# samson6460/tf2_YOLO

Hardware: AMD Instinct MI355X
Metric: images/sec training YOLOv3 416x416 bs=32/GPU (higher is better)
Workload: dtype f32-storage/fp16x2-mfma

## Files before the change

include/yolo_hip.h:

```cpp
#ifndef YOLO_HIP_H_
#define YOLO_HIP_H_

#include <stddef.h>
#include <stdint.h>

#ifdef __cplusplus
extern "C" {
#endif

typedef enum yolo_status {
  YOLO_OK = 0,
  YOLO_ERR_INVALID_ARG = -1,
  YOLO_ERR_LAUNCH = -2,
  YOLO_ERR_WORKSPACE = -3
} yolo_status;

enum { YOLO_ACT_LINEAR = 0, YOLO_ACT_LEAKY = 1, YOLO_ACT_MISH = 2 };
enum { YOLO_HEAD_V3 = 3, YOLO_HEAD_V2 = 2, YOLO_HEAD_V1 = 1, YOLO_HEAD_V4 = 4 };
enum { YOLO_NMS_HARD = 1, YOLO_NMS_SOFT = 2, YOLO_NMS_DIOU = 3 };

const char* yolo_last_error(void);
int yolo_abi_version(void);
int yolo_device_available(void);
int yolo_mfma_probe(const void* operands_f16, float* sink, int workgroups, int iters, double* flops_host, void* stream);

enum { YOLO_OPT_CONV_WIN = 0, YOLO_OPT_STAMPS = 1, YOLO_OPT_CONV_SK = 2, YOLO_OPT_CONV_PATCH = 5, YOLO_OPT_WGRAD_WIN = 6,
       YOLO_OPT_NMS_WALK = 7 ,
       YOLO_OPT_AB = 8  };
int yolo_set_option(int key, int value);
size_t yolo_conv_workspace_bytes(void);
int yolo_set_conv_workspace(void* p, size_t bytes, void* stream);
int yolo_set_debug_buffer(void* p, size_t bytes);

typedef struct yolo_conv_desc {
  int N, H, W, Cin;
  int Cout, kh, kw;
  int Ho, Wo;
  int sh, sw;
  int pad_t, pad_l;
} yolo_conv_desc;

#define YOLO_BN_STAT_SLOTS 64
#define YOLO_BN_RED_SLOTS 512
#define YOLO_SPLIT_BATCH_UNITS 4

int yolo_conv2d_fwd(const yolo_conv_desc* d, const float* x, const float* w,
                    const float* bias, float* y, double* stats, void* stream);
int yolo_conv2d_fwd_absmax(const yolo_conv_desc* d, const float* x, const float* w, const float* bias,
                           float* y, double* stats, unsigned* absmax, void* stream);

int yolo_conv2d_dgrad(const yolo_conv_desc* d, const float* dy, const float* wT,
                      float* dx, int accumulate, void* stream);

int yolo_conv2d_wgrad(const yolo_conv_desc* d, const float* x, const float* dy,
                      float* dw, float* dbias, void* stream);

int yolo_conv2d_wgrad_bias(const float* dy, long long P, int Cout, float* dbias, void* stream);

int yolo_filter_transpose(const float* w, float* wT, int Cout, int taps, int Cin, void* stream);

size_t yolo_planes_bytes(long long rows, int C);
int yolo_split_planes(const float* x, long long rows, int C, void* planes, void* stream);
int yolo_split_planes_padded(const float* x, long long rows, int C_src, int C, void* planes, void* stream);

int yolo_split_planes_batch(const void* jobs, int njobs, long long total_blocks, void* stream);
int yolo_filter_transpose_batch(const void* jobs, int njobs, long long total_blocks, void* stream);

int yolo_conv2d_fwd_planes(const yolo_conv_desc* d, const void* x_planes, const void* w_planes,
                           const float* bias, float* y, double* stats, unsigned* absmax, void* stream);
int yolo_conv2d_dgrad_planes(const yolo_conv_desc* d, const void* dy_planes, const void* wT_planes,
                             float* dx, int accumulate, void* stream);
enum { YOLO_EPI_NONE = 0, YOLO_EPI_AFFINE = 1, YOLO_EPI_AFFINE_LEAKY = 2, YOLO_EPI_AFFINE_MISH = 3 };
int yolo_conv2d_fwd_planes_epi(const yolo_conv_desc* d, const void* x_planes, const void* w_planes, const float* bias,
                               int epilogue, const float* scale, const float* shift, const float* residual, float* y,
                               unsigned* absmax, void* stream);
int yolo_split_planes_absmax(const float* x, long long rows, int C, const unsigned* absmax, const float* extra_bound,
                             void* planes, float* out_bound, void* stream);
#define YOLO_INFER_BOUND_WORDS 4096
int yolo_conv_pred_bound(const float* w, int Cout, int kdim, const float* scale, const float* shift, const float* bias,
                         float* pred2, void* stream);
int yolo_conv2d_fwd_infer_unit(const yolo_conv_desc* d, const void* x_planes, const void* w_planes, const float* bias,
                               int epilogue, const float* scale, const float* shift, const float* residual, float* y,
                               unsigned* absmax, const float* pred2, const void* in_bound, int in_n,
                               const void* residual_bound, int residual_n, void* out_planes, unsigned* out_words,
                               float* out_bound, int* out_n_host, void* stream);
int yolo_fold_bound(const void* words, int n, float* out_bound, void* stream);
int yolo_absmax_words(const float* x, long long n, unsigned* words, int* n_words_host, void* stream);
int yolo_stem_filter_prep(const float* w, const float* bias, float* wt, void* stream);
int yolo_stem_fwd_infer_unit(const yolo_conv_desc* d, const float* x, const float* wt, int epilogue, const float* scale,
                             const float* shift, const float* pred2, const void* in_bound, int in_n, float* y,
                             void* out_planes, unsigned* out_words, int* out_n_host, void* stream);
int yolo_split_planes_concat(const float* const* srcs_host, const int* channels_host, const float* const* bounds_host,
                             int nsrc, long long rows, void* planes, float* dst32, float* out_bound, void* stream);
int yolo_split_planes_concat_ex(const float* const* srcs_host, const int* channels_host, const float* const* bounds_host,
                                const int* bound_words_host, const int* upsample_host, int H, int W, int nsrc,
                                long long rows, void* planes, float* dst32, float* out_bound, void* stream);
int yolo_conv2d_fwd_head_unit(const yolo_conv_desc* d, const void* x_planes, const void* w_planes, const float* bias,
                              int A, int C, int version, const float* anchors, float* t, float* y, void* stream);
int yolo_conv2d_wgrad_planes(const yolo_conv_desc* d, const void* x_planes, const void* dy_planes,
                             float* dw, void* stream);

size_t yolo_wgrad_workspace_bytes(void);
int yolo_set_wgrad_workspace(void* p, size_t bytes);


int yolo_bn_stats(const float* x, long long P, int C, double* stats, void* stream);

int yolo_bn_finalize(double* stats, long long P, int C, const float* gamma, const float* beta,
                     float eps, float momentum, int unbiased_moving_var,
                     float* moving_mean, float* moving_var,
                     float* scale, float* shift, float* save_mean, float* save_invstd,
                     void* stream);

int yolo_bn_fold_inference(int C, const float* gamma, const float* beta,
                           const float* moving_mean, const float* moving_var, float eps,
                           float* scale, float* shift, void* stream);

int yolo_bn_act_fwd(const float* x, long long P, int C, const float* scale, const float* shift,
                    int act, const float* residual, float* out, void* stream);

int yolo_bn_act_bwd_reduce(const float* x, const float* dout, long long P, int C,
                           const float* scale, const float* shift,
                           const float* save_mean, const float* save_invstd,
                           int act, double* red, void* stream);
int yolo_bn_act_bwd_apply(const float* x, const float* dout, long long P, int C,
                          const float* gamma, const float* scale, const float* shift,
                          const float* save_mean, const float* save_invstd,
                          int act, double* red, float* dgamma, float* dbeta,
                          float* dx, void* stream);

int yolo_bn_finalize_bound(double* stats, long long P, int C, const float* gamma, const float* beta, float eps,
                           float momentum, int unbiased_moving_var, float* moving_mean, float* moving_var,
                           float* scale, float* shift, float* save_mean, float* save_invstd,
                           const unsigned* absmax, unsigned* bound, void* stream);
int yolo_bn_finalize_offset(double* stats, long long P, int C, const float* gamma, const float* beta, float eps,
                            float momentum, int unbiased_moving_var, float* moving_mean, float* moving_var, float* scale,
                            float* shift, float* save_mean, float* save_invstd, const unsigned* absmax, unsigned* bound,
                            const float* mean_offset, void* stream);
int yolo_bn_infer_bound(int C, const float* scale, const float* shift, const unsigned* absmax,
                        unsigned* bound, void* stream);
int yolo_bn_act_fwd_planes(const float* x, long long P, int C, const float* scale, const float* shift,
                           int act, const float* residual, float* out, void* planes,
                           const unsigned* bn_bound, const float* residual_bound, float* out_bound,
                           void* stream);
int yolo_bn_act_maxpool2x2_fwd(const float* y, int N, int Ho, int Wo, int C, const float* scale, const float* shift,
                               int act, float* out, int* argmax, void* planes, const unsigned* bn_bound,
// ... 3 lines not shown
                               float* out_bound, void* stream);
int yolo_bn_act_bwd_reduce_bound(const float* x, const float* dout, long long P, int C, const float* scale,
                                 const float* shift, const float* save_mean, const float* save_invstd,
                                 int act, double* red, unsigned* bound_aux, void* stream);
size_t yolo_stem_bwd_scratch_bytes(void);
int yolo_stem_bn_bwd_wgrad(const yolo_conv_desc* d, const float* y, const float* dout, const float* image, const float* scale,
                           const float* shift, const float* save_mean, const float* save_invstd, int act, const double* red,
                           float* dgamma, float* dbeta, float* dw, void* scratch, size_t scratch_bytes, void* stream);
int yolo_bn_act_bwd_apply_planes(const float* x, const float* dout, long long P, int C, const float* gamma,
                                 const float* scale, const float* shift, const float* save_mean,
                                 const float* save_invstd, int act, double* red, float* dgamma, float* dbeta,
                                 float* dx, void* planes, const unsigned* bound_aux, void* stream);
int yolo_bn_act_bwd_reduce_bound_ld(const float* x, const float* dout, long long ld_dout, long long P, int C,
                                    const float* scale, const float* shift, const float* save_mean,
                                    const float* save_invstd, int act, double* red, unsigned* bound_aux, void* stream);
#define YOLO_BN_FOLD_TICKET_WORDS 36
int yolo_bn_act_bwd_reduce_fold_ld(const float* x, const float* dout, long long ld_dout, long long P, int C,
                                   const float* scale, const float* shift, const float* save_mean,
                                   const float* save_invstd, int act, double* red, unsigned* bound_aux,
                                   unsigned* tickets, void* stream);
int yolo_bn_act_bwd_apply_planes_ld(const float* x, const float* dout, long long ld_dout, long long P, int C,
                                    const float* gamma, const float* scale, const float* shift, const float* save_mean,
                                    const float* save_invstd, int act, double* red, float* dgamma, float* dbeta,
                                    float* dx, void* planes, const unsigned* bound_aux, void* stream);

int yolo_bnred_slots_cap(const yolo_conv_desc* d);
int yolo_conv2d_dgrad_planes_bnred(const yolo_conv_desc* d, const void* dy_planes, const void* wT_planes, float* dx,
                                   int accumulate, const float* y, const float* scale, const float* shift,
                                   const float* save_mean, const float* save_invstd, int act, float* partials,
                                   int slots_cap, unsigned* bound_aux, int* nslots, void* stream);
int yolo_bn_act_bwd_sum_partials(const float* partials, int nslots, long long P, int C, const float* scale, double* red,
                                 unsigned* bound_aux, void* stream);

int yolo_act_fwd(const float* x, long long n, int act, float* out, void* stream);
int yolo_act_bwd(const float* x, const float* dout, long long n, int act, float* dx, void* stream);

int yolo_copy_channels_in(const float* src, long long P, int Csrc, float* dst, int Cdst,
                          int c_off, void* stream);
int yolo_copy_channels_out(const float* src, long long P, int Csrc, int c_off, float* dst,
                           int Cdst, int accumulate, void* stream);
int yolo_upsample2x_fwd(const float* x, int N, int H, int W, int C, float* y, int Cy, int c_off,
                        void* stream);
int yolo_upsample2x_bwd(const float* dy, int N, int H, int W, int C, int Cy, int c_off, float* dx,
                        int accumulate, void* stream);
int yolo_axpy(float* a, const float* b, long long n, void* stream);
int yolo_maxpool_fwd(const float* x, int N, int H, int W, int C, int k, int s, int pad_t, int pad_l,
                     int Ho, int Wo, float* y, int Cy, int c_off, int* argmax, void* stream);
int yolo_maxpool_bwd(const float* dy, int N, int Ho, int Wo, int C, int Cy, int c_off,
                     const int* argmax, float* dx, void* stream);
int yolo_maxpool_bwd_same(const float* dy, int N, int H, int W, int C, int Cy, int c_off, const int* argmax, int k,
                          int pad_t, int pad_l, float* dx, void* stream);
int yolo_maxpool2x2_bwd(const float* dy, int N, int Ho, int Wo, int C, const int* argmax, float* dx, int accumulate,
                        void* stream);
int yolo_space_to_depth2_fwd(const float* x, int N, int H, int W, int C, float* y, int Cy, int c_off,
                             void* stream);
int yolo_space_to_depth2_bwd(const float* dy, int N, int H, int W, int C, int Cy, int c_off, float* dx,
                             int accumulate, void* stream);

int yolo_head_act_fwd(const float* t, long long P, int A, int C, int version,
                      const float* anchors, float* y, void* stream);
int yolo_head_act_bwd(const float* y, const float* dy, long long P, int A, int C, int version,
                      const float* anchors, float* dt, float* danchors, void* stream);

typedef struct yolo_loss_cfg {
  int version;
  int N, gh, gw, A, C;
  float anchors[32];
  int   use_anchors;
  float binary_weight;
  float loss_weight[4];
  float ignore_thresh;
  int   use_focal_loss;
  float focal_gamma;
  int   use_scale;
  float wh_reg_weight;
  float truth_thresh;
  float label_smooth;
} yolo_loss_cfg;

size_t yolo_loss_workspace_bytes(const yolo_loss_cfg* cfg);
int yolo_loss_fwd_bwd(const yolo_loss_cfg* cfg, const float* y_true, const float* y_pred,
                      double* loss_out, float* dpred, float grad_scale,
                      void* workspace, size_t workspace_bytes, void* stream);

int yolo_metrics(const yolo_loss_cfg* cfg, const float* y_true, const float* y_pred,
                 float recall_thresh, double* out, void* stream);

int yolo_adam_step(float* p, float* g, float* m, float* v, long long n, float lr, float beta1,
                   float beta2, float eps, int step, float grad_scale, int zero_grad, void* stream);
float yolo_adam_lr_t(float lr, float beta1, float beta2, int step);
int yolo_adam_step_dev(float* p, float* g, float* m, float* v, long long n, const float* hyper, int zero_grad, void* stream);
int yolo_sgd_step(float* p, float* g, long long n, float lr, float grad_scale, int zero_grad,
                  void* stream);
int yolo_fill(float* p, long long n, float value, void* stream);

size_t yolo_grad_sqnorm_workspace_bytes(int n_chunks);
int yolo_grad_sqnorm(const float* g, const long long* chunk_off, const int* chunk_len, int n_chunks,
                     const int* var_first, int n_vars, double* var_sq, double* total_sq, void* workspace,
                     size_t workspace_bytes, void* stream);
int yolo_clip_factors(const double* var_sq, int n_vars, const double* total_sq, const double* total_sq_extra,
                      const float* hyper, int mode, float* factors, float* norm_out, void* stream);
int yolo_adam_step_clip(float* p, float* g, float* m, float* v, float* vhat, const long long* chunk_off,
                        const int* chunk_len, const int* chunk_var, int n_chunks, const float* hyper,
                        const float* factors, int clip_mode, int zero_grad, void* stream);
int yolo_sgd_step_clip(float* p, float* g, float* accum, int nesterov, const long long* chunk_off,
                       const int* chunk_len, const int* chunk_var, int n_chunks, const float* hyper,
                       const float* factors, int clip_mode, int zero_grad, void* stream);

int yolo_decode_level(const float* pred, int gh, int gw, int A, int C, int version,
                      float threshold, double* rows_out, int max_rows, int* count,
                      void* workspace, size_t workspace_bytes, void* stream);
int yolo_decode_level_f64(const double* pred, int gh, int gw, int A, int C, int version,
                          double threshold, double* rows_out, int max_rows, int* count,
                          void* workspace, size_t workspace_bytes, void* stream);
size_t yolo_decode_workspace_bytes(int gh, int gw, int A, int C);

size_t yolo_nms_workspace_bytes(int n, int class_num);
int yolo_nms(const double* rows, int n, int class_num, int mode, double nms_threshold,
             double conf_threshold, double sigma, unsigned char* keep_out,
             void* workspace, size_t workspace_bytes, void* stream);
int yolo_nms_select(const double* rows, int n, int class_num, int mode, double nms_threshold, double conf_threshold,
                    double sigma, unsigned char* keep_out, double* rows_out, int* count_out, void* workspace,
                    size_t workspace_bytes, void* stream);

int yolo_cal_iou(const void* xywh_true, const void* xywh_pred, void* out, void* out2, int is_f64, int mode, int ndim,
                 const long long* shape_host, const long long* true_strides_host, const long long* pred_strides_host,
                 double grid_w, double grid_h, void* stream);


int yolo_match_detections(const double* gt_rows, int ngt, const double* det_rows, int ndet, int class_num,
                          double iou_threshold, int* best_gt, unsigned char* matched, double* best_iou,
                          unsigned char* gt_flags, long long* class_counts, void* stream);

int yolo_rank_desc(const double* key, const int* segment, int n, int* rank, void* stream);

size_t yolo_pr_curve_workspace_bytes(int n, int num_gts);
int yolo_pr_curve(const double* joint, const int* gt_id, const unsigned char* matched, int n, int num_gts,
                  int precision_mode, void* workspace, size_t workspace_bytes, double* precision,
                  double* recall, void* stream);

int yolo_allreduce_bucket(void* rccl_comm, float* grads, long long count, void* stream);

int yolo_encode_labels(const double* boxes, const int* cls, const int* first, int N, double img_h, double img_w,
                       int gh, int gw, int C, double* label64, float* label32, void* stream);
int yolo_down2xlabel(const double* label_in, int N, int gh, int gw, int ch, double* label_out, float* out32,
                     void* stream);

#ifdef __cplusplus
}
#endif
#endif
```

tf2_yolo_amd/_lib.py:

```python
import ctypes
import os
from ctypes import (POINTER, Structure, c_char_p, c_double, c_float, c_int, c_longlong,
                    c_size_t, c_void_p)

from . import tape as _tape

_HERE = os.path.dirname(os.path.abspath(__file__))
LIB_PATH = os.path.join(_HERE, "libyolo_hip.so")

ACT_LINEAR, ACT_LEAKY, ACT_MISH = 0, 1, 2
NMS_HARD, NMS_SOFT, NMS_DIOU = 1, 2, 3


class YoloHipError(RuntimeError):
    pass


class ConvDesc(Structure):
    _fields_ = [(n, c_int) for n in
                ("N", "H", "W", "Cin", "Cout", "kh", "kw", "Ho", "Wo", "sh", "sw", "pad_t", "pad_l")]


class LossCfg(Structure):
    _fields_ = [("version", c_int), ("N", c_int), ("gh", c_int), ("gw", c_int), ("A", c_int),
                ("C", c_int), ("anchors", c_float * 32), ("use_anchors", c_int),
                ("binary_weight", c_float), ("loss_weight", c_float * 4),
                ("ignore_thresh", c_float), ("use_focal_loss", c_int), ("focal_gamma", c_float),
                ("use_scale", c_int), ("wh_reg_weight", c_float), ("truth_thresh", c_float),
                ("label_smooth", c_float)]


_P = c_void_p
_LL = c_longlong
SIGNATURES = {
    "yolo_last_error": (c_char_p, []),
    "yolo_abi_version": (c_int, []),
    "yolo_device_available": (c_int, []),
    "yolo_set_option": (c_int, [c_int, c_int]),
    "yolo_mfma_probe": (c_int, [_P, _P, c_int, c_int, POINTER(c_double), _P]),
    "yolo_set_debug_buffer": (c_int, [_P, c_size_t]),
    "yolo_encode_labels": (c_int, [_P, _P, _P, c_int, c_double, c_double, c_int, c_int, c_int, _P, _P, _P]),
    "yolo_down2xlabel": (c_int, [_P, c_int, c_int, c_int, c_int, _P, _P, _P]),
    "yolo_conv_workspace_bytes": (c_size_t, []),
    "yolo_set_conv_workspace": (c_int, [_P, c_size_t, _P]),
    "yolo_conv2d_fwd": (c_int, [POINTER(ConvDesc), _P, _P, _P, _P, _P, _P]),
    "yolo_conv2d_dgrad": (c_int, [POINTER(ConvDesc), _P, _P, _P, c_int, _P]),
    "yolo_conv2d_wgrad": (c_int, [POINTER(ConvDesc), _P, _P, _P, _P, _P]),
    "yolo_conv2d_wgrad_bias": (c_int, [_P, _LL, c_int, _P, _P]),
    "yolo_filter_transpose": (c_int, [_P, _P, c_int, c_int, c_int, _P]),
    "yolo_planes_bytes": (c_size_t, [_LL, c_int]),
    "yolo_split_planes": (c_int, [_P, _LL, c_int, _P, _P]),
    "yolo_split_planes_padded": (c_int, [_P, _LL, c_int, c_int, _P, _P]),
    "yolo_split_planes_batch": (c_int, [_P, c_int, _LL, _P]),
    "yolo_filter_transpose_batch": (c_int, [_P, c_int, _LL, _P]),
    "yolo_conv2d_fwd_planes": (c_int, [POINTER(ConvDesc), _P, _P, _P, _P, _P, _P, _P]),
    "yolo_stem_bwd_scratch_bytes": (c_size_t, []),
    "yolo_stem_bn_bwd_wgrad": (c_int, [POINTER(ConvDesc), _P, _P, _P, _P, _P, _P, _P, c_int, _P, _P, _P, _P, _P, c_size_t, _P]),
    "yolo_conv2d_fwd_planes_epi": (c_int, [POINTER(ConvDesc), _P, _P, _P, c_int, _P, _P, _P, _P, _P, _P]),
    "yolo_split_planes_absmax": (c_int, [_P, _LL, c_int, _P, _P, _P, _P, _P]),
    "yolo_conv_pred_bound": (c_int, [_P, c_int, c_int, _P, _P, _P, _P, _P]),
    "yolo_conv2d_fwd_infer_unit": (c_int, [POINTER(ConvDesc), _P, _P, _P, c_int, _P, _P, _P, _P, _P, _P, _P, c_int, _P, c_int,
                                           _P, _P, _P, POINTER(c_int), _P]),
    "yolo_fold_bound": (c_int, [_P, c_int, _P, _P]),
    "yolo_absmax_words": (c_int, [_P, _LL, _P, POINTER(c_int), _P]),
    "yolo_stem_filter_prep": (c_int, [_P, _P, _P, _P]),
    "yolo_stem_fwd_infer_unit": (c_int, [POINTER(ConvDesc), _P, _P, c_int, _P, _P, _P, _P, c_int, _P, _P, _P, POINTER(c_int), _P]),
    "yolo_split_planes_concat": (c_int, [POINTER(c_void_p), POINTER(c_int), POINTER(c_void_p), c_int, _LL, _P, _P, _P, _P]),
    "yolo_split_planes_concat_ex": (c_int, [POINTER(c_void_p), POINTER(c_int), POINTER(c_void_p), POINTER(c_int), POINTER(c_int),
                                            c_int, c_int, c_int, _LL, _P, _P, _P, _P]),
    "yolo_conv2d_fwd_head_unit": (c_int, [POINTER(ConvDesc), _P, _P, _P, c_int, c_int, c_int, _P, _P, _P, _P]),
    "yolo_conv2d_fwd_absmax": (c_int, [POINTER(ConvDesc), _P, _P, _P, _P, _P, _P, _P]),
    "yolo_conv2d_dgrad_planes": (c_int, [POINTER(ConvDesc), _P, _P, _P, c_int, _P]),
    "yolo_conv2d_wgrad_planes": (c_int, [POINTER(ConvDesc), _P, _P, _P, _P]),
    "yolo_wgrad_workspace_bytes": (c_size_t, []),
    "yolo_set_wgrad_workspace": (c_int, [_P, c_size_t]),
    "yolo_bn_stats": (c_int, [_P, _LL, c_int, _P, _P]),
    "yolo_bn_finalize": (c_int, [_P, _LL, c_int, _P, _P, c_float, c_float, c_int, _P, _P, _P, _P, _P, _P, _P]),
    "yolo_bn_fold_inference": (c_int, [c_int, _P, _P, _P, _P, c_float, _P, _P, _P]),
    "yolo_bn_act_fwd": (c_int, [_P, _LL, c_int, _P, _P, c_int, _P, _P, _P]),
    "yolo_bn_act_bwd_reduce": (c_int, [_P, _P, _LL, c_int, _P, _P, _P, _P, c_int, _P, _P]),
    "yolo_bn_act_bwd_apply": (c_int, [_P, _P, _LL, c_int, _P, _P, _P, _P, _P, c_int, _P, _P, _P, _P, _P]),
    "yolo_bn_act_fwd_planes": (c_int, [_P, _LL, c_int, _P, _P, c_int, _P, _P, _P, _P, _P, _P, _P]),
    "yolo_bn_act_fwd_res_planes": (c_int, [_P, _LL, c_int, _P, _P, c_int, _P, _P, _P, _P, _P, _P]),
    "yolo_bn_act_bwd_apply_planes": (c_int, [_P, _P, _LL, c_int, _P, _P, _P, _P, _P, c_int, _P, _P, _P, _P, _P, _P,
                                             _P]),
    "yolo_bn_infer_bound": (c_int, [c_int, _P, _P, _P, _P, _P]),
    "yolo_bn_finalize_bound": (c_int, [_P, _LL, c_int, _P, _P, c_float, c_float, c_int, _P, _P, _P, _P, _P, _P, _P,
                                       _P, _P]),
    "yolo_bn_finalize_offset": (c_int, [_P, _LL, c_int, _P, _P, c_float, c_float, c_int, _P, _P, _P, _P, _P, _P, _P,
                                        _P, _P, _P]),
    "yolo_bn_act_bwd_reduce_bound": (c_int, [_P, _P, _LL, c_int, _P, _P, _P, _P, c_int, _P, _P, _P]),
    "yolo_bn_act_bwd_reduce_bound_ld": (c_int, [_P, _P, _LL, _LL, c_int, _P, _P, _P, _P, c_int, _P, _P, _P]),
    "yolo_bn_act_bwd_reduce_fold_ld": (c_int, [_P, _P, _LL, _LL, c_int, _P, _P, _P, _P, c_int, _P, _P, _P, _P]),
    "yolo_bn_act_bwd_apply_planes_ld": (c_int, [_P, _P, _LL, _LL, c_int, _P, _P, _P, _P, _P, c_int, _P, _P, _P, _P, _P, _P,
                                                _P]),
    "yolo_bnred_slots_cap": (c_int, [POINTER(ConvDesc)]),
    "yolo_conv2d_dgrad_planes_bnred": (c_int, [POINTER(ConvDesc), _P, _P, _P, c_int, _P, _P, _P, _P, _P, c_int, _P, c_int, _P,
                                               POINTER(c_int), _P]),
    "yolo_bn_act_bwd_sum_partials": (c_int, [_P, c_int, _LL, c_int, _P, _P, _P, _P]),
    "yolo_allreduce_bucket": (c_int, [_P, _P, _LL, _P]),
    "yolo_act_fwd": (c_int, [_P, _LL, c_int, _P, _P]),
    "yolo_act_bwd": (c_int, [_P, _P, _LL, c_int, _P, _P]),
    "yolo_copy_channels_in": (c_int, [_P, _LL, c_int, _P, c_int, c_int, _P]),
    "yolo_copy_channels_out": (c_int, [_P, _LL, c_int, c_int, _P, c_int, c_int, _P]),
    "yolo_upsample2x_fwd": (c_int, [_P, c_int, c_int, c_int, c_int, _P, c_int, c_int, _P]),
    "yolo_upsample2x_bwd": (c_int, [_P, c_int, c_int, c_int, c_int, c_int, c_int, _P, c_int, _P]),
    "yolo_axpy": (c_int, [_P, _P, _LL, _P]),
    "yolo_maxpool_fwd": (c_int, [_P, c_int, c_int, c_int, c_int, c_int, c_int, c_int, c_int, c_int, c_int,
                                 _P, c_int, c_int, _P, _P]),
    "yolo_maxpool_bwd": (c_int, [_P, c_int, c_int, c_int, c_int, c_int, c_int, _P, _P, _P]),
    "yolo_maxpool2x2_bwd": (c_int, [_P, c_int, c_int, c_int, c_int, _P, _P, c_int, _P]),
    "yolo_bn_act_maxpool2x2_fwd": (c_int, [_P, c_int, c_int, c_int, c_int, _P, _P, c_int, _P, _P, _P, _P, _P, _P]),
    "yolo_maxpool_bwd_same": (c_int, [_P, c_int, c_int, c_int, c_int, c_int, c_int, _P, c_int, c_int, c_int, _P, _P]),
    "yolo_space_to_depth2_fwd": (c_int, [_P, c_int, c_int, c_int, c_int, _P, c_int, c_int, _P]),
    "yolo_space_to_depth2_bwd": (c_int, [_P, c_int, c_int, c_int, c_int, c_int, c_int, _P, c_int, _P]),
    "yolo_head_act_fwd": (c_int, [_P, _LL, c_int, c_int, c_int, _P, _P, _P]),
    "yolo_head_act_bwd": (c_int, [_P, _P, _LL, c_int, c_int, c_int, _P, _P, _P, _P]),
    "yolo_loss_workspace_bytes": (c_size_t, [POINTER(LossCfg)]),
    "yolo_loss_fwd_bwd": (c_int, [POINTER(LossCfg), _P, _P, _P, _P, c_float, _P, c_size_t, _P]),
    "yolo_metrics": (c_int, [POINTER(LossCfg), _P, _P, c_float, _P, _P]),
    "yolo_adam_step": (c_int, [_P, _P, _P, _P, _LL, c_float, c_float, c_float, c_float, c_int, c_float, c_int, _P]),
    "yolo_adam_lr_t": (c_float, [c_float, c_float, c_float, c_int]),
    "yolo_adam_step_dev": (c_int, [_P, _P, _P, _P, _LL, _P, c_int, _P]),
    "yolo_sgd_step": (c_int, [_P, _P, _LL, c_float, c_float, c_int, _P]),
    "yolo_fill": (c_int, [_P, _LL, c_float, _P]),
    "yolo_grad_sqnorm_workspace_bytes": (c_size_t, [c_int]),
    "yolo_grad_sqnorm": (c_int, [_P, _P, _P, c_int, _P, c_int, _P, _P, _P, c_size_t, _P]),
    "yolo_clip_factors": (c_int, [_P, c_int, _P, _P, _P, c_int, _P, _P, _P]),
    "yolo_adam_step_clip": (c_int, [_P, _P, _P, _P, _P, _P, _P, _P, c_int, _P, _P, c_int, c_int, _P]),
    "yolo_sgd_step_clip": (c_int, [_P, _P, _P, c_int, _P, _P, _P, c_int, _P, _P, c_int, c_int, _P]),
    "yolo_decode_level": (c_int, [_P, c_int, c_int, c_int, c_int, c_int, c_float, _P, c_int, _P, _P, c_size_t, _P]),
    "yolo_decode_level_f64": (c_int, [_P, c_int, c_int, c_int, c_int, c_int, c_double, _P, c_int, _P, _P,
                                      c_size_t, _P]),
    "yolo_decode_workspace_bytes": (c_size_t, [c_int, c_int, c_int, c_int]),
    "yolo_nms_workspace_bytes": (c_size_t, [c_int, c_int]),
    "yolo_cal_iou": (c_int, [_P, _P, _P, _P, c_int, c_int, c_int, POINTER(c_longlong), POINTER(c_longlong),
                             POINTER(c_longlong), c_double, c_double, _P]),
    "yolo_match_detections": (c_int, [_P, c_int, _P, c_int, c_int, c_double, _P, _P, _P, _P, _P, _P]),
    "yolo_rank_desc": (c_int, [_P, _P, c_int, _P, _P]),
    "yolo_pr_curve_workspace_bytes": (c_size_t, [c_int, c_int]),
    "yolo_pr_curve": (c_int, [_P, _P, _P, c_int, c_int, c_int, _P, c_size_t, _P, _P, _P]),
    "yolo_nms": (c_int, [_P, c_int, c_int, c_int, c_double, c_double, c_double, _P, _P, c_size_t, _P]),
    "yolo_nms_select": (c_int, [_P, c_int, c_int, c_int, c_double, c_double, c_double, _P, _P, _P, _P, c_size_t, _P]),
}

_lib = None

_QUERIES = {"yolo_last_error", "yolo_abi_version", "yolo_bnred_slots_cap", "yolo_device_available", "yolo_conv_workspace_bytes", "yolo_planes_bytes",
            "yolo_stem_bwd_scratch_bytes", "yolo_loss_workspace_bytes", "yolo_decode_workspace_bytes",
            "yolo_nms_workspace_bytes", "yolo_pr_curve_workspace_bytes", "yolo_wgrad_workspace_bytes", "yolo_adam_lr_t",
            "yolo_grad_sqnorm_workspace_bytes",
            "yolo_set_option", "yolo_set_debug_buffer", "yolo_set_conv_workspace", "yolo_set_wgrad_workspace"}


class _Recorded:
    __slots__ = ("f", "name")

    def __init__(self, f, name):
        self.f, self.name = f, name

    def __call__(self, *a):
        rc = self.f(*a)
        if _tape.ACTIVE is not None:
            _tape.ACTIVE.c(self.f, a, self.name)
        return rc


class _Lib:

    def __init__(self, cdll):
        self._cdll = cdll

    def __getattr__(self, name):
        f = getattr(self._cdll, name)
        if name not in _QUERIES and name in SIGNATURES:
            f = _Recorded(f, name)
        setattr(self, name, f)
        return f


def load():
    global _lib
    if _lib is not None:
        return _lib
    if not os.path.exists(LIB_PATH):
        raise YoloHipError(
            f"{LIB_PATH} not found: build it with `make` (or __graft_entry__.build()); "
            "there is no CPU fallback for the product path")
    import torch
    try:
        lib = ctypes.CDLL(LIB_PATH)
    except OSError as e:
        raise YoloHipError(f"cannot load {LIB_PATH}: {e}") from e
    for name, (res, args) in SIGNATURES.items():
        try:
            fn = getattr(lib, name)
        except AttributeError as e:
            raise YoloHipError(f"{LIB_PATH} does not export {name}") from e
        fn.restype = res
        fn.argtypes = args
    _lib = _Lib(lib)
    return _lib
# ... 7 lines not shown
```

tf2_yolo_amd/capture.py:

```python
import torch

from ._lib import YoloHipError


_LEAKED = []


class _StaticInputs:

    def __init__(self, x, y_list):
        self.x = x.clone()
        self.ys = [y.clone() for y in y_list]
        self._last = [(x, x._version)] + [(y, y._version) for y in y_list]

    def load(self, x, y_list):
        for i, (dst, src) in enumerate(zip([self.x] + self.ys, [x] + list(y_list))):
            last, ver = self._last[i]
            if src is last and src._version == ver:
                continue
            dst.copy_(src, non_blocking=True)
            self._last[i] = (src, src._version)


class StepGraphs:

    def __init__(self, model, x, y_list):
        self.model = model
        self.key = self.key_of(model, x)
        net = model.net
        opt = model.optimizer
        if not getattr(opt, "capturable", False):
            raise YoloHipError("this optimizer has no capturable form")
        self.inputs = _StaticInputs(x, y_list)
        self.x, self.ys = self.inputs.x, self.inputs.ys
        self.segments = []
        opt._hyper_buffers()
        net.mark_params_changed()
        torch.cuda.synchronize()
        self._capture(net, opt)

    @staticmethod
    def key_of(model, x):
        return (tuple(x.shape), getattr(model.net, "alloc_gen", 0), tuple(id(l) for l in model.loss), id(model.optimizer),
                id(model._reducer), model.net.anchors_trainable)

    def _capture(self, net, opt):
        model = self.model
        red = model._reducer if (model._reducer is not None and model._reducer.active) else None
        pool = torch.cuda.graph_pool_handle()
        stream = torch.cuda.Stream()
        stream.wait_stream(torch.cuda.current_stream())
        state = {"g": None}

        def begin():
            g = torch.cuda.CUDAGraph()
            g.capture_begin(pool=pool, capture_error_mode="thread_local")
            state["g"] = g

        def end(action):
            state["g"].capture_end()
            self.segments.append((state["g"], action))
            state["g"] = None

        net._dyp_events = [None, None]
        net._wp_event = net._wT_event = None
        old_hook, old_overlap = net.grad_ready_hook, net._overlap_wgrad
        net._overlap_wgrad = False
        if red is not None:
            index = model._dp_unit_index

            def cut_hook(u):
                for b in red.closes[index[id(u)]]:
                    net._join_wgrad()
                    net._dyp_events = [None, None]
                    end(("reduce", b))
                    begin()
            net.grad_ready_hook = cut_hook
        try:
            with torch.cuda.stream(stream):
                begin()
                outs = net.forward(self.x, training=True)
                for i, (o, yt) in enumerate(zip(outs, self.ys)):
                    model.loss[i].fwd_bwd(yt, o, grad_scale=1.0, dpred=model._dpred[i], loss_out=model._loss_bufs[i])
                net.backward(model._dpred)
                net._dyp_events = [None, None]
                if red is not None:
                    end(("finish",))
                    begin()
                opt.step_captured()
                end(None)
        except Exception:
            _LEAKED.extend(g for g, _ in self.segments)
            if state["g"] is not None:
                _LEAKED.append(state["g"])
                try:
                    if net._wgrad_stream is not None:
                        torch.cuda.current_stream().wait_stream(net._wgrad_stream)
                    state["g"].capture_end()
                except Exception:
                    pass
            self.segments = []
            net._dyp_events = [None, None]
            net._wp_event = net._wT_event = None
            net._wgrad_pending = False
            raise
        finally:
            net.grad_ready_hook = old_hook
            net._overlap_wgrad = old_overlap
        torch.cuda.current_stream().wait_stream(stream)
        net.mark_params_changed()

    def replay(self, x, y_list):
        model, net, opt = self.model, self.model.net, self.model.optimizer
        red = model._reducer if (model._reducer is not None and model._reducer.active) else None
        self.inputs.load(x, y_list)
        opt.refresh_hyper(grad_scale=(1.0 / red.world) if red is not None else 1.0)
        for g, action in self.segments:
            g.replay()
            if action is None:
                continue
            if action[0] == "reduce":
                red.reduce_bucket(action[1])
            else:
                if net.anchors_trainable and red.world > 1:
                    import torch.distributed as dist
                    dist.all_reduce(net.anchor_grads, group=red.pg)
                red.finish()
        net.mark_params_changed()
        return model._loss_bufs


class StepTape:

    def __init__(self, model, x, y_list):
        from . import tape as tape_mod
        self.model = model
        self.key = StepGraphs.key_of(model, x)
        opt, net = model.optimizer, model.net
        if not getattr(opt, "capturable", False):
            raise YoloHipError("this optimizer has no capturable form")
        self.inputs = _StaticInputs(x, y_list)
        self.x, self.ys = self.inputs.x, self.inputs.ys
        opt._hyper_buffers()
        red = model._reducer if (model._reducer is not None and model._reducer.active) else None
        net._dyp_events = [None, None]
        net.mark_params_changed()
        self.tape = tape_mod.Tape()
        opt.refresh_hyper(grad_scale=(1.0 / red.world) if red is not None else 1.0)
        tape_mod.ACTIVE = self.tape
        try:
            outs = net.forward(self.x, training=True)
            for i, (o, yt) in enumerate(zip(outs, self.ys)):
                model.loss[i].fwd_bwd(yt, o, grad_scale=1.0, dpred=model._dpred[i], loss_out=model._loss_bufs[i])
            net.backward(model._dpred)
            if red is not None:
                if net.anchors_trainable and red.world > 1:
                    import torch.distributed as dist
                    tape_mod.host_call(lambda: dist.all_reduce(net.anchor_grads, group=red.pg))
                tape_mod.host_call(red.finish)
            opt.step_captured()
        finally:
            tape_mod.ACTIVE = None
        net.mark_params_changed()

    def replay(self, x, y_list):
        model, net, opt = self.model, self.model.net, self.model.optimizer
        red = model._reducer if (model._reducer is not None and model._reducer.active) else None
        self.inputs.load(x, y_list)
        opt.refresh_hyper(grad_scale=(1.0 / red.world) if red is not None else 1.0)
        self.tape.replay()
        net.mark_params_changed()
        return model._loss_bufs
```

tf2_yolo_amd/csrc/conv.hip:

```cpp
#include "conv_args.hpp"
#include <cstdlib>
#include <type_traits>

namespace yolo {

template <int BM, int BN, int WGM, int WGN, bool FLAT>
__global__ __launch_bounds__(256) void gather_conv_kernel(const GatherConvArgs a) {
  constexpr int BK = 32;
  constexpr int LD = BK + 4;
  constexpr int TM = BM / WGM / 32;
  constexpr int TN = BN / WGN / 32;
  constexpr int AR = BM / 32;
  constexpr int BR = BN / 32;
  static_assert(WGM * WGN == 4, "4 waves per block");
  static_assert(TM >= 1 && TN >= 1, "wave tile");

  extern __shared__ __attribute__((aligned(16))) float smem[];
  constexpr int BUF = (BM + BN) * LD;

  const int tid = threadIdx.x;
  const int lane = tid & 63;
  const int wave = tid >> 6;
  const int wm = wave / WGN, wn = wave % WGN;

// ... 935 lines not shown
    C += channels_host[i];
  }
  YOLO_REQUIRE((C % 16) == 0, "split_planes_concat: the concatenated channel count must be a multiple of 16");
  return launch_split_planes_concat(srcs_host, channels_host, bounds_host, nsrc, rows, planes, dst32, out_bound,
                                    as_stream(stream));
}

extern "C" int yolo_split_planes_concat_ex(const float* const* srcs_host, const int* channels_host,
                                           const float* const* bounds_host, const int* bound_words_host,
                                           const int* upsample_host, int H, int W, int nsrc, long long rows, void* planes,
                                           float* dst32, float* out_bound, void* stream) {
  YOLO_REQUIRE(srcs_host && channels_host && bounds_host && planes && nsrc >= 1 && nsrc <= 4 && rows > 0,
               "split_planes_concat: 1..4 sources, non-null tables");
  int C = 0;
  bool any_up = false;
  for (int i = 0; i < nsrc; ++i) {
    YOLO_REQUIRE(srcs_host[i] && bounds_host[i] && channels_host[i] > 0 && (channels_host[i] % 8) == 0,
                 "split_planes_concat: every source needs a pointer, a bound and a channel count that is a multiple of 8");
    YOLO_REQUIRE(bound_words_host == nullptr || (bound_words_host[i] >= 1 && bound_words_host[i] <= YOLO_INFER_BOUND_WORDS),
                 "split_planes_concat: a bound is 1..%d words", YOLO_INFER_BOUND_WORDS);
    any_up = any_up || (upsample_host != nullptr && upsample_host[i] != 0);
    C += channels_host[i];
  }
  YOLO_REQUIRE((C % 16) == 0, "split_planes_concat: the concatenated channel count must be a multiple of 16");
  YOLO_REQUIRE(!any_up || (H > 0 && W > 0 && (H % 2) == 0 && (W % 2) == 0 && rows % ((long long)H * W) == 0),
               "split_planes_concat: an upsampled source needs even H, W with rows = N * H * W (H=%d W=%d rows=%lld)", H, W, rows);
  return launch_split_planes_concat(srcs_host, channels_host, bounds_host, nsrc, rows, planes, dst32, out_bound,
                                    as_stream(stream), bound_words_host, upsample_host, H, W);
}

extern "C" int yolo_conv2d_fwd_head_unit(const yolo_conv_desc* d, const void* x_planes, const void* w_planes,
                                         const float* bias, int A, int C, int version, const float* anchors, float* t,
                                         float* y, void* stream) {
  if (int rc = validate_desc(d)) return rc;
  YOLO_REQUIRE(x_planes && w_planes && t && y && A > 0 && C > 0, "conv_fwd_head_unit: bad args");
  YOLO_REQUIRE(d->Cout == A * (5 + C), "conv_fwd_head_unit: Cout = %d is not A (5 + C) = %d", d->Cout, A * (5 + C));
  GatherConvArgs a{};
  a.src = reinterpret_cast<const float*>(x_planes);
  a.wgt = reinterpret_cast<const float*>(w_planes);
  a.bias = bias;
  a.dst = t;
  fill_fwd_args(d, a);
  YOLO_REQUIRE(gather_planes_supported(a), "conv_fwd_head_unit: needs Cin %% 16 == 0 and Cout >= 32");
  if ((version == YOLO_HEAD_V3 || version == YOLO_HEAD_V4) && anchors != nullptr) {
    a.head_y = y;
    a.head_anchors = anchors;
    a.head_A = A;
    a.head_C = C;
    if (conv_small_head_supported(a)) {
      int nwg = 0;
      return launch_conv_small(a, as_stream(stream), &nwg);
    }
    a.head_y = nullptr;
  }
  if (int rc = launch_gather_planes(a, as_stream(stream))) return rc;
  return yolo_head_act_fwd(t, (long long)d->N * d->Ho * d->Wo, A, C, version, anchors, y, stream);
}

extern "C" size_t yolo_planes_bytes(long long rows, int C) {
  if (rows <= 0 || C <= 0 || (C % 16) != 0) return 0;
  return (size_t)planes_bytes(rows, C);
}

extern "C" int yolo_split_planes_batch(const void* jobs, int njobs, long long total_blocks, void* stream) {
  YOLO_REQUIRE(jobs, "split_planes_batch: null job table");
  return launch_split_planes_batch(jobs, njobs, total_blocks, as_stream(stream));
}

extern "C" int yolo_filter_transpose_batch(const void* jobs, int njobs, long long total_blocks, void* stream) {
  YOLO_REQUIRE(jobs, "filter_transpose_batch: null job table");
  return launch_filter_transpose_batch(jobs, njobs, total_blocks, as_stream(stream));
}

extern "C" int yolo_split_planes(const float* x, long long rows, int C, void* planes, void* stream) {
  YOLO_REQUIRE(x && planes, "split_planes: null pointer");
  return launch_split_planes(x, rows, C, planes, as_stream(stream));
}

extern "C" int yolo_split_planes_padded(const float* x, long long rows, int C_src, int C, void* planes, void* stream) {
  YOLO_REQUIRE(x && planes, "split_planes_padded: null pointer");
  return launch_split_planes_padded(x, rows, C_src, C, planes, as_stream(stream));
}

struct BnRedArgs {
  const float* y;
  const float* scale;
  const float* shift;
  const float* mean;
  const float* invstd;
  int act;
  float* part;
  int cap;
  unsigned* aux;
  int nslots;
};
static void set_bnred(GatherConvArgs& a, const BnRedArgs* b) {
  if (b == nullptr) return;
  a.bwd_y = b->y; a.bwd_scale = b->scale; a.bwd_shift = b->shift; a.bwd_mean = b->mean; a.bwd_invstd = b->invstd;
  a.bwd_act = b->act; a.bwd_part = b->part; a.bwd_cap = b->cap; a.bwd_aux = b->aux;
}

static int dgrad_impl(const yolo_conv_desc* d, const float* dy, const float* wT, float* dx, int accumulate,
                      void* stream, bool planes, BnRedArgs* bnred = nullptr) {
  if (int rc = validate_desc(d)) return rc;
  YOLO_REQUIRE(dy && wT && dx, "conv_dgrad: null pointer");
  const bool flat = (d->Cout % 32) != 0;
  YOLO_REQUIRE(!flat || (d->kh == 1 && d->kw == 1 && d->sh == 1 && d->sw == 1),
               "conv_dgrad: Cout %% 32 != 0 only supported for 1x1 stride-1 (head) convs");
  static const bool fuse_classes = env_int("YOLO_DGRAD_CLASSES", 1) != 0;
  if (planes && fuse_classes && d->sh * d->sw > 1 && d->sh * d->sw <= 4) {
    GatherConvArgs a{};
    a.src = dy;
    a.wgt = wT;
    a.dst = dx;
    a.N = d->N; a.Hs = d->Ho; a.Ws = d->Wo; a.Cs = d->Cout;
    a.sy = 1; a.sx = 1;
    a.Hd = d->H; a.Wd = d->W; a.Cd = d->Cin;
    a.osy = d->sh; a.osx = d->sw;
    a.Cout = d->Cin;
    a.ldw = d->kh * d->kw * d->Cout;
    a.accumulate = accumulate;
    a.kw = 1;
    int nt = 0, nc = 0;
    bool ok = true;
    for (int py = 0; py < d->sh && ok; ++py)
      for (int px = 0; px < d->sw && ok; ++px) {
        ClassGeom& c = a.cls[nc++];
        c.Hg = (d->H - py + d->sh - 1) / d->sh;
        c.Wg = (d->W - px + d->sw - 1) / d->sw;
        c.M = (long long)d->N * c.Hg * c.Wg;
        c.ooy = py; c.oox = px; c.tap0 = nt; c.ntaps = 0;
        for (int r = 0; r < d->kh; ++r) {
          const int ty = py + d->pad_t - r;
          if (((ty % d->sh) + d->sh) % d->sh != 0) continue;
          for (int s = 0; s < d->kw; ++s) {
            const int tx = px + d->pad_l - s;
            if (((tx % d->sw) + d->sw) % d->sw != 0) continue;
            a.taps[nt++] = Tap{ty / d->sh, tx / d->sw, (r * d->kw + s) * d->Cout};
            ++c.ntaps;
          }
        }
        if (c.ntaps == 0 || c.Hg <= 0 || c.Wg <= 0) ok = false;
      }
    if (ok) {
      a.ncls = nc;
      a.M = a.cls[0].M; a.Hg = a.cls[0].Hg; a.Wg = a.cls[0].Wg; a.ooy = 0; a.oox = 0; a.ntaps = a.cls[0].ntaps;
      YOLO_REQUIRE(gather_planes_supported(a), "conv_dgrad_planes: needs Cout %% 16 == 0 and Cin >= 32");
      set_bnred(a, bnred);
      const int rc = launch_gather_planes(a, as_stream(stream));
      if (bnred != nullptr) bnred->nslots = a.bwd_nslots;
      return rc;
    }
  }
  YOLO_REQUIRE(bnred == nullptr || d->sh * d->sw == 1,
               "conv_dgrad_planes_bnred: a strided data gradient needs its parity classes in one launch");
  for (int py = 0; py < d->sh; ++py) {
    for (int px = 0; px < d->sw; ++px) {
      GatherConvArgs a{};
      a.src = dy;
      a.wgt = wT;
      a.bias = nullptr;
      a.dst = dx;
      a.N = d->N; a.Hs = d->Ho; a.Ws = d->Wo; a.Cs = d->Cout;
      a.Hg = (d->H - py + d->sh - 1) / d->sh;
      a.Wg = (d->W - px + d->sw - 1) / d->sw;
      if (a.Hg <= 0 || a.Wg <= 0) continue;
// ... 154 lines not shown
```

tf2_yolo_amd/csrc/conv_args.hpp:

```cpp
#pragma once
#include "common.hpp"

namespace yolo {

constexpr int MAX_TAPS = 49;

struct Tap {
  int oy, ox, woff;
};

struct ClassGeom {
  long long M;
  int Hg, Wg, ooy, oox, tap0, ntaps;
};

struct GatherConvArgs {
  const float* src;
  const float* wgt;
  const float* bias;
  float* dst;
  double* stats;
  unsigned* absmax;
  long long M;
  int N, Hs, Ws, Cs;
// ... 9 lines not shown
  unsigned src_bytes, wgt_bytes;
  int zero_blk_src, zero_blk_wgt;
  int nt_store;
  int vec_store;
  int kc;
  int dbg;
  const float* epi_scale;
  const float* epi_shift;
  const float* epi_res;
  int epi_act;
  unsigned char* out_planes;
  const float* pl_pred;
  const unsigned* pl_in_bound;
  const unsigned* pl_res_bound;
  int pl_in_n, pl_res_n;
  unsigned* pl_out_words;
  float* head_y;
  const float* head_anchors;
  int head_A, head_C;
  int sk_grid;
  int tile_order;
  float* sk_slabs;
  unsigned* sk_tickets;
  int split_parts;
  int ncls;
  ClassGeom cls[4];
  unsigned long long* stamps;
  const float* bwd_y;
  const float* bwd_scale;
  const float* bwd_shift;
  const float* bwd_mean;
  const float* bwd_invstd;
  float* bwd_part;
  unsigned* bwd_aux;
  int bwd_act;
  int bwd_nslots;
  int bwd_cap;
  Tap taps[MAX_TAPS];
};

#define YOLO_BNRED_CHECK(a)                                                                                          \
  if ((a).bwd_y != nullptr && (a).bwd_nslots > (a).bwd_cap) {                                                        \
    set_error("conv_dgrad(bn reduce): %d partial slots needed, room for %d", (a).bwd_nslots, (a).bwd_cap);           \
    return YOLO_ERR_INVALID_ARG;                                                                                     \
  }

__device__ __forceinline__ int xcd_remap(int bid, int nblocks) {
  const int xcd = bid & 7, idx = bid >> 3;
  const int q = nblocks >> 3, r = nblocks & 7;
  const int start = (xcd < r) ? xcd * (q + 1) : r * (q + 1) + (xcd - r) * q;
  return start + idx;
}


struct WgradArgs {
  const float* src;
  const float* dy;
  float* dw;
  long long M;
  int N, Hs, Ws, Cs;
  int Hg, Wg;
  int sy, sx;
  int Cout, ldw;
  int ntaps;
  int kw, pad_t, pad_l;
  int tiles_co, tiles_j;
  int nblocks;
  long long chunk;
  unsigned src_bytes, dy_bytes;
  int zero_blk_src, zero_blk_dy;
  float* slabs;
  int splits;
};

int launch_gather_split(GatherConvArgs& a, hipStream_t st);
bool gather_split_supported(const GatherConvArgs& a);
long long planes_bytes(long long rows, int C);
int launch_split_planes(const float* x, long long rows, int C, void* planes, hipStream_t st);
int launch_split_planes_absmax(const float* x, long long rows, int C, const unsigned* absmax, const float* extra_bound, int extra_n,
                               void* planes, float* out_bound, hipStream_t st);
int launch_split_planes_concat(const float* const* xs, const int* Cs, const float* const* bounds, int nsrc, long long rows,
                               void* planes, float* dst32, float* out_bound, hipStream_t st,
                               const int* bound_words = nullptr, const int* upsample = nullptr, int H = 0, int W = 0);
int launch_split_planes_padded(const float* x, long long rows, int Csrc, int C, void* planes, hipStream_t st);
int launch_split_planes_batch(const void* jobs, int njobs, long long total_blocks, hipStream_t st);
int launch_filter_transpose_batch(const void* jobs, int njobs, long long total_blocks, hipStream_t st);
int launch_gather_planes(GatherConvArgs& a, hipStream_t st);
bool conv_small_supported(const GatherConvArgs& a);
bool conv_small_head_supported(const GatherConvArgs& a);
int launch_conv_small(GatherConvArgs& a, hipStream_t st, int* nwg);
bool gather_planes_supported(const GatherConvArgs& a);
int conv_split_parts(const GatherConvArgs& a, long long nb, int bm, int min_cb, int idle_div);
int launch_split_reduce(GatherConvArgs& a, int bm, hipStream_t st);
float* conv_split_slabs();
int launch_conv_win(GatherConvArgs& a, int variant, hipStream_t st);
bool conv_win_supported(const GatherConvArgs& a);
enum { OPT_CONV_WIN = 0, OPT_STAMPS = 1, OPT_CONV_SK = 2, OPT_DBG = 3, OPT_TILE_ORDER = 4, OPT_CONV_PATCH = 5, OPT_WGRAD_WIN = 6, OPT_NMS_WALK = 7, OPT_EXP = 8, OPT_COUNT = 16 };
int set_conv_workspace(void* p, size_t bytes, hipStream_t st);
extern void* g_dbg_buf;
extern size_t g_dbg_bytes;
extern int g_opt[OPT_COUNT];
void init_options();
int launch_wgrad_planes(WgradArgs& a, hipStream_t st);
bool wgrad_planes_supported(const WgradArgs& a);
int launch_wgrad_win(WgradArgs& a, hipStream_t st);
bool wgrad_win_supported(const WgradArgs& a);
constexpr size_t WGRAD_WS_COLSUM_BYTES = 1 << 20;
void* wgrad_workspace(size_t* bytes);
bool stem_fwd_supported(const yolo_conv_desc* d);
struct StemEpiArgs {
  const float* scale;
  const float* shift;
  int act;
  void* planes;
  const float* pred;
  const unsigned* in_words;
  int in_n;
  unsigned* out_words;
};
bool stem_infer_supported(const yolo_conv_desc* d);
int launch_stem_filter_prep(const float* w, const float* bias, float* wt, hipStream_t st);
int launch_absmax_words(const float* x, long long n, unsigned* words, int* n_words, hipStream_t st);
int launch_stem_infer(const yolo_conv_desc* d, const float* x, const float* wt, float* y, const StemEpiArgs& e, int* out_n,
                      hipStream_t st);
size_t stem_bwd_scratch_bytes();
int launch_stem_bn_bwd_wgrad(const yolo_conv_desc* d, const float* y, const float* dout, const float* img, const float* scale,
                             const float* shift, const float* smean, const float* sinv, int act, const double* redsum,
                             float* dgamma, float* dbeta, float* dw, float* scratch, size_t scratch_bytes, hipStream_t st);
int launch_stem_fwd(const yolo_conv_desc* d, const float* x, const float* w, const float* bias, float* y, double* stats,
                    unsigned* absmax, hipStream_t st);
int launch_wgrad_split(WgradArgs& a, hipStream_t st);
bool wgrad_split_supported(const WgradArgs& a);

}
```

tf2_yolo_amd/csrc/conv_planes.hip:

```cpp
#include "planes_epilogue.hpp"
#include <algorithm>
#include <cstdlib>
#include <type_traits>

namespace yolo {

__global__ __launch_bounds__(256) void planes_amax_kernel(const float* __restrict__ x, long long n4,
                                                         unsigned* __restrict__ header) {
  float m = 0.f;
  for (long long i = (long long)blockIdx.x * 256 + threadIdx.x; i < n4; i += (long long)gridDim.x * 256) {
    const f32x4 v = reinterpret_cast<const f32x4*>(x)[i];
    m = fmaxf(fmaxf(m, fmaxf(fabsf(v[0]), fabsf(v[1]))), fmaxf(fabsf(v[2]), fabsf(v[3])));
  }
#pragma unroll
  for (int o = 32; o > 0; o >>= 1) m = fmaxf(m, __shfl_xor(m, o, 64));
  __shared__ float wmax[4];
  if ((threadIdx.x & 63) == 0) wmax[threadIdx.x >> 6] = m;
  __syncthreads();
  if (threadIdx.x == 0) {
    m = fmaxf(fmaxf(wmax[0], wmax[1]), fmaxf(wmax[2], wmax[3]));
    if (__builtin_bit_cast(unsigned, m) > *reinterpret_cast<volatile unsigned*>(header))
      atomicMax(header, __builtin_bit_cast(unsigned, m));
  }
}
// ... 679 lines not shown
  const BatchJob j = jobs[find_job(jobs, njobs, blockIdx.x)];
  const float* x = reinterpret_cast<const float*>(j.src);
  unsigned char* out = reinterpret_cast<unsigned char*>(j.dst);
  const long long rows = j.a;
  const int C = (int)j.b;
  unsigned* header = reinterpret_cast<unsigned*>(out + planes_body_bytes(rows, C));
  const unsigned bound = j.c != 0 ? *reinterpret_cast<const unsigned*>(j.c) : header[0];
  const float sc = planes_scale_from_bound(bound);
  const long long rows_padded = ((rows + 15) / 16 + 1) * 16;
  if ((long long)blockIdx.x == j.first_block && threadIdx.x == 0) {
    header[0] = bound;
    reinterpret_cast<float*>(header)[1] = sc;
    reinterpret_cast<float*>(header)[2] = 1.f / sc;
  }
  const BatchPos p = batch_pos(j);
  if (!p.live) return;
  f32x4 v[BATCH_UNITS][2];
#pragma unroll
  for (int u = 0; u < BATCH_UNITS; ++u) {
    const long long row = p.row0 + 16 * u;
    v[u][0] = v[u][1] = f32x4{0.f, 0.f, 0.f, 0.f};
    if (row < rows) {
      const float* q = x + row * C + p.g * 8;
      v[u][0] = *reinterpret_cast<const f32x4*>(q);
      v[u][1] = *reinterpret_cast<const f32x4*>(q + 4);
    }
  }
#pragma unroll
  for (int u = 0; u < BATCH_UNITS; ++u) {
    const long long row = p.row0 + 16 * u;
    if (row >= rows_padded) continue;
    const Planes8 s8 = split8(v[u][0], v[u][1], sc);
    unsigned char* o = out + planes_unit_offset(row, p.g, C);
    *reinterpret_cast<u32x4*>(o) = s8.h;
    *reinterpret_cast<u32x4*>(o + 512) = s8.l;
  }
}

__global__ __launch_bounds__(256) void filter_transpose_batch_kernel(const BatchJob* __restrict__ jobs, int njobs) {
  __shared__ float tile[32][33];
  const BatchJob j = jobs[find_job(jobs, njobs, blockIdx.x)];
  const float* w = reinterpret_cast<const float*>(j.src);
  float* wT = reinterpret_cast<float*>(j.dst);
  const int Cout = (int)j.a, taps = (int)j.b, Cin = (int)j.c;
  const int bx = (Cin + 31) / 32, by = (Cout + 31) / 32;
  const int lb = (int)((long long)blockIdx.x - j.first_block);
  const int t = lb / (bx * by);
  const int rem = lb - t * (bx * by);
  const int co0 = (rem / bx) * 32, ci0 = (rem % bx) * 32;
  const int tx = threadIdx.x & 31, ty = threadIdx.x >> 5;
  for (int r = ty; r < 32; r += 8) {
    const int co = co0 + r, ci = ci0 + tx;
    tile[r][tx] = (co < Cout && ci < Cin) ? w[((long long)co * taps + t) * Cin + ci] : 0.f;
  }
  __syncthreads();
  for (int r = ty; r < 32; r += 8) {
    const int ci = ci0 + r, co = co0 + tx;
    if (ci < Cin && co < Cout) wT[((long long)ci * taps + t) * Cout + co] = tile[tx][r];
  }
}

int launch_split_planes_batch(const void* jobs, int njobs, long long total_blocks, hipStream_t st) {
  if (njobs <= 0 || total_blocks <= 0 || total_blocks > 0x7fffffffLL) {
    set_error("split_planes_batch: bad job table");
    return YOLO_ERR_INVALID_ARG;
  }
  const BatchJob* jb = reinterpret_cast<const BatchJob*>(jobs);
  hipLaunchKernelGGL(planes_header_clear_batch_kernel, dim3((njobs + 255) / 256), dim3(256), 0, st, jb, njobs);
  hipLaunchKernelGGL(planes_amax_batch_kernel, dim3((unsigned)total_blocks), dim3(256), 0, st, jb, njobs);
  hipLaunchKernelGGL(split_planes_batch_kernel, dim3((unsigned)total_blocks), dim3(256), 0, st, jb, njobs);
  return check_launch("split_planes_batch_kernel");
}

int launch_filter_transpose_batch(const void* jobs, int njobs, long long total_blocks, hipStream_t st) {
  if (njobs <= 0 || total_blocks <= 0 || total_blocks > 0x7fffffffLL) {
    set_error("filter_transpose_batch: bad job table");
    return YOLO_ERR_INVALID_ARG;
  }
  hipLaunchKernelGGL(filter_transpose_batch_kernel, dim3((unsigned)total_blocks), dim3(256), 0, st,
                     reinterpret_cast<const BatchJob*>(jobs), njobs);
  return check_launch("filter_transpose_batch_kernel");
}

int launch_split_planes_padded(const float* x, long long rows, int Csrc, int C, void* planes, hipStream_t st) {
  if (C % 16 != 0 || rows <= 0 || Csrc <= 0 || Csrc > C || C - Csrc >= 16) {
    set_error("split_planes_padded: need 0 < Csrc <= C < Csrc + 16, C %% 16 == 0, rows > 0");
    return YOLO_ERR_INVALID_ARG;
  }
  const long long rows_padded = ((rows + 15) / 16 + 1) * 16;
  const long long blocks = (rows_padded * (C / 8) + 255) / 256;
  if (blocks > 0x7fffffffLL) {
    set_error("split_planes_padded: tensor too large");
    return YOLO_ERR_INVALID_ARG;
  }
  unsigned char* out = reinterpret_cast<unsigned char*>(planes);
  unsigned* header = reinterpret_cast<unsigned*>(out + planes_body_bytes(rows, C));
  if (hipMemsetAsync(header, 0, 16, st) != hipSuccess) {
    set_error("split_planes_padded: hipMemsetAsync failed");
    return YOLO_ERR_LAUNCH;
  }
  const long long n = rows * Csrc, n4 = n / 4;
  if (n4 > 0) hipLaunchKernelGGL(planes_amax_kernel, dim3(stream_grid(n4, 256)), dim3(256), 0, st, x, n4, header);
  if (n > 4 * n4)
    hipLaunchKernelGGL(planes_amax_scalar_kernel, dim3(1), dim3(256), 0, st, x + 4 * n4, n - 4 * n4, header);
  hipLaunchKernelGGL(split_planes_padded_kernel, dim3((unsigned)blocks), dim3(256), 0, st, x, rows, Csrc, C, out,
                     rows_padded);
  return check_launch("split_planes_padded_kernel");
}

int launch_split_planes_absmax(const float* x, long long rows, int C, const unsigned* absmax, const float* extra_bound, int extra_n,
                               void* planes, float* out_bound, hipStream_t st) {
  if (C % 16 != 0 || rows <= 0) {
    set_error("split_planes_absmax: C %% 16 != 0 or rows <= 0");
    return YOLO_ERR_INVALID_ARG;
  }
  const long long rows_padded = ((rows + 15) / 16 + 1) * 16;
  const long long blocks = ((rows_padded / 16 + SPLIT_BLOCKS_PER_WG - 1) / SPLIT_BLOCKS_PER_WG) * ((C / 8 + 15) / 16);
  if (blocks > 0x7fffffffLL) {
    set_error("split_planes_absmax: tensor too large");
    return YOLO_ERR_INVALID_ARG;
  }
  hipLaunchKernelGGL(split_planes_absmax_kernel, dim3((unsigned)blocks), dim3(256), 0, st, x, rows, C, absmax, extra_bound,
                     extra_n, reinterpret_cast<unsigned char*>(planes), rows_padded, out_bound);
  return check_launch("split_planes_absmax_kernel");
}

int launch_split_planes(const float* x, long long rows, int C, void* planes, hipStream_t st) {
  if (C % 16 != 0 || rows <= 0) {
    set_error("split_planes: C %% 16 != 0 or rows <= 0");
    return YOLO_ERR_INVALID_ARG;
  }
  const long long rows_padded = ((rows + 15) / 16 + 1) * 16;
  const long long blocks = ((rows_padded / 16 + SPLIT_BLOCKS_PER_WG - 1) / SPLIT_BLOCKS_PER_WG) * ((C / 8 + 15) / 16);
  if (blocks > 0x7fffffffLL) {
    set_error("split_planes: tensor too large");
    return YOLO_ERR_INVALID_ARG;
  }
  unsigned char* out = reinterpret_cast<unsigned char*>(planes);
  unsigned* header = reinterpret_cast<unsigned*>(out + planes_body_bytes(rows, C));
  if (hipMemsetAsync(header, 0, 16, st) != hipSuccess) {
    set_error("split_planes: hipMemsetAsync failed");
    return YOLO_ERR_LAUNCH;
  }
  const long long n4 = rows * (C / 4);
  hipLaunchKernelGGL(planes_amax_kernel, dim3(stream_grid(n4, 256)), dim3(256), 0, st, x, n4, header);
  hipLaunchKernelGGL(split_planes_kernel, dim3((unsigned)blocks), dim3(256), 0, st, x, rows, C, out, rows_padded);
  return check_launch("split_planes_kernel");
}

}
```

tf2_yolo_amd/csrc/loss.hip:

```cpp
#include "common.hpp"
#include "conv_args.hpp"
#include <cfloat>
#include <cstdlib>

namespace yolo {

constexpr float LEPS = 1e-7f;
constexpr float ONE_M_EPS = (float)(1.0 - 1e-7);

struct D4 {
  float v;
  float d[4];
};
__device__ __forceinline__ D4 dconst(float v) { return D4{v, {0.f, 0.f, 0.f, 0.f}}; }
__device__ __forceinline__ D4 dvar(float v, int i) {
  D4 r = dconst(v);
  r.d[i] = 1.f;
  return r;
}
__device__ __forceinline__ D4 operator+(const D4& a, const D4& b) {
  D4 r{a.v + b.v, {}};
  for (int i = 0; i < 4; ++i) r.d[i] = a.d[i] + b.d[i];
  return r;
}
__device__ __forceinline__ D4 operator-(const D4& a, const D4& b) {
  D4 r{a.v - b.v, {}};
  for (int i = 0; i < 4; ++i) r.d[i] = a.d[i] - b.d[i];
  return r;
}
__device__ __forceinline__ D4 operator*(const D4& a, const D4& b) {
  D4 r{a.v * b.v, {}};
  for (int i = 0; i < 4; ++i) r.d[i] = a.d[i] * b.v + a.v * b.d[i];
  return r;
}
__device__ __forceinline__ D4 operator/(const D4& a, const D4& b) {
  D4 r{a.v / b.v, {}};
  for (int i = 0; i < 4; ++i) r.d[i] = a.d[i] / b.v - (a.v / b.v) / b.v * b.d[i];
  return r;
}
__device__ __forceinline__ D4 dmax(const D4& x, const D4& y) { return (x.v >= y.v) ? x : y; }
__device__ __forceinline__ D4 dmin(const D4& x, const D4& y) { return (x.v <= y.v) ? x : y; }
__device__ __forceinline__ D4 dsq(const D4& a) {
  D4 r{a.v * a.v, {}};
  for (int i = 0; i < 4; ++i) r.d[i] = 2.f * a.v * a.d[i];
  return r;
}
__device__ __forceinline__ D4 datan(const D4& a) {
  D4 r{atanf(a.v), {}};
  const float g = 1.f / (1.f + a.v * a.v);
  for (int i = 0; i < 4; ++i) r.d[i] = g * a.d[i];
  return r;
}

struct IouOut {
  D4 iou;
  D4 ciou;
};

template <bool CIOU>
__device__ __forceinline__ IouOut iou_dual(const float* T, const float* P, float gw, float gh) {
  const D4 px = dvar(P[0], 0), py = dvar(P[1], 1), pw = dvar(P[2], 2), ph = dvar(P[3], 3);
  const D4 cx = px / dconst(gw), cy = py / dconst(gh);
  const float tcx = T[0] / gw, tcy = T[1] / gh, tw = T[2], th = T[3];
  const float thw = tw / 2.f, thh = th / 2.f;
  const float tminx = tcx - thw, tmaxx = tcx + thw, tminy = tcy - thh, tmaxy = tcy + thh;
  const D4 hw = pw / dconst(2.f), hh = ph / dconst(2.f);
  const D4 minx = cx - hw, maxx = cx + hw, miny = cy - hh, maxy = cy + hh;
  const D4 iminx = dmax(minx, dconst(tminx)), iminy = dmax(miny, dconst(tminy));
  const D4 imaxx = dmin(maxx, dconst(tmaxx)), imaxy = dmin(maxy, dconst(tmaxy));
  const D4 iw = dmax(imaxx - iminx, dconst(0.f)), ih = dmax(imaxy - iminy, dconst(0.f));
  const D4 inter = iw * ih;
  const float tarea = tw * th;
  const D4 parea = pw * ph;
  const D4 uni = parea + dconst(tarea) - inter;
  IouOut o;
  o.iou = inter / (uni + dconst(LEPS));
  o.ciou = o.iou;
  if constexpr (CIOU) {
    const D4 eminx = dmin(minx, dconst(tminx)), eminy = dmin(miny, dconst(tminy));
    const D4 emaxx = dmax(maxx, dconst(tmaxx)), emaxy = dmax(maxy, dconst(tmaxy));
    const D4 ewx = emaxx - eminx, ewy = emaxy - eminy;
    const D4 c2 = dsq(ewx) + dsq(ewy);
    const D4 rho2 = dsq(dconst(tcx) - cx) + dsq(dconst(tcy) - cy);
    const float atan_t = atanf(tw / (th + LEPS));
    const D4 atan_p = datan(pw / (ph + dconst(LEPS)));
    const D4 v = dconst((float)(4.0 / (M_PI * M_PI))) * dsq(dconst(atan_t) - atan_p);
    const D4 alpha = v / (dconst(1.f) - o.iou + v);
    o.ciou = o.iou - rho2 / c2 - alpha * v;
  }
  return o;
}

struct LossParams {
  yolo_loss_cfg c;
  long long cells;
  float inv_n;
  int* dec;
};

template <int VER>
__device__ __forceinline__ float loss_channel(const yolo_loss_cfg& c, const int b, const int k, const float p, const float tk_cur,
                                              const float t4, const float (&Tb)[4], const float iou_b, const float d0,
                                              const float d1, const float d2, const float d3, const float an, const float cb,
                                              const float r_b, double (&part)[7]) {
  (void)b;
  const float tbk = (k == 0) ? Tb[0] : (k == 1) ? Tb[1] : (k == 2) ? Tb[2] : Tb[3];
  float obj, noobj;
  if (VER == 1) {
    obj = t4 * r_b;
    noobj = 1.f - obj;
  } else {
    obj = t4 * r_b;
    if (VER == 4 && c.truth_thresh < 1.f) obj = obj + ((iou_b > c.truth_thresh) ? 1.f : 0.f) * (1.f - obj);
    noobj = (1.f - obj) * ((iou_b < c.ignore_thresh) ? 1.f : 0.f);
  }
  float g = 0.f;

  if (k < 4) {
    const float dIk = (k == 0) ? d0 : (k == 1) ? d1 : (k == 2) ? d2 : d3;
    if (VER == 2 || VER == 3) {
      const float s = (VER == 2 || c.use_scale) ? (2.f - Tb[2] * Tb[3]) : 1.f;
      if (k < 2) {
        const float diff = tbk - p;
        const float l = obj * s * (diff * diff);
        part[1] += (double)l;
        part[0] += (double)c.loss_weight[0] * (double)l;
        g = -2.f * c.loss_weight[0] * obj * s * diff;
      } else {
        const float tl = logf(fmaxf(tbk / an, LEPS));
        const float pl = logf(p / an);
        const float diff = tl - pl;
        const float l = obj * s * (diff * diff);
        const float reg = pl * pl;
        part[2] += (double)l;
        part[6] += (double)reg;
        part[0] += (double)c.loss_weight[1] * (double)l + 0.01 * (double)reg;
        g = (-2.f * c.loss_weight[1] * obj * s * diff + 0.02f * pl) / p;
      }
    } else if (VER == 4) {
      g = -c.loss_weight[0] * obj * dIk;
      if (k >= 2) {
        const float pl = logf(p / an);
        const float reg = pl * pl;
        part[6] += (double)reg;
        part[0] += (double)c.wh_reg_weight * (double)reg;
        g += 2.f * c.wh_reg_weight * pl / p;
      }
    } else {
      g = 2.f * c.loss_weight[2] * obj * (iou_b - cb) * dIk;
      if (k < 2) {
        const float diff = tbk - p;
        const float l = obj * (diff * diff);
        part[1] += (double)l;
        part[0] += (double)c.loss_weight[0] * (double)l;
        g += -2.f * c.loss_weight[0] * obj * diff;
      } else {
        const float tq = sqrtf(fmaxf(tbk, LEPS));
        const float pq = sqrtf(fmaxf(p, LEPS));
        const float diff = tq - pq;
        const float l = obj * (diff * diff);
        part[2] += (double)l;
        part[0] += (double)c.loss_weight[1] * (double)l;
        if (p >= LEPS) g += -2.f * c.loss_weight[1] * obj * diff * (0.5f / pq);
      }
    }
  } else if (k == 4) {
    if (VER == 1) {
      const float e = iou_b - p;
      const float lo = obj * (e * e);
      const float ln = noobj * (p * p);
      part[3] += (double)lo;
      part[4] += (double)ln;
      part[0] += (double)c.loss_weight[2] * ((double)lo + (double)c.binary_weight * (double)ln);
      g = c.loss_weight[2] * (-2.f * obj * e + 2.f * c.binary_weight * noobj * p);
    } else if (VER == 2 || (VER == 3 && !c.use_focal_loss)) {
      const float lo = obj * ((1.f - p) * (1.f - p));
      const float ln = noobj * (p * p);
      part[3] += (double)lo;
      part[4] += (double)ln;
      part[0] += (double)c.loss_weight[2] * ((double)lo + (double)c.binary_weight * (double)ln);
      g = c.loss_weight[2] * (-2.f * obj * (1.f - p) + 2.f * c.binary_weight * noobj * p);
    } else if (VER == 3) {
      const float cc = fminf(fmaxf(p, LEPS), ONE_M_EPS);
      const float pass = (p >= LEPS && p <= ONE_M_EPS) ? 1.f : 0.f;
      const float gm = c.focal_gamma;
      const bool g2 = gm == 2.f;
      const float a1 = g2 ? (1.f - cc) * (1.f - cc) : powf(1.f - cc, gm), l1 = logf(cc);
      const float a0 = g2 ? cc * cc : powf(cc, gm), l0 = logf(1.f - cc);
      const float lo = -obj * a1 * l1;
      const float ln = -noobj * a0 * l0;
      part[3] += (double)lo;
      part[4] += (double)ln;
      part[0] += (double)c.loss_weight[2] * ((double)lo + (double)c.binary_weight * (double)ln);
      const float d1 = -obj * (-gm * (g2 ? (1.f - cc) : powf(1.f - cc, gm - 1.f)) * l1 + a1 / cc);
      const float d0 = -noobj * (gm * (g2 ? cc : powf(cc, gm - 1.f)) * l0 - a0 / (1.f - cc));
      g = c.loss_weight[2] * (d1 + c.binary_weight * d0) * pass;
    } else {
      const float cc = fminf(fmaxf(p, LEPS), ONE_M_EPS);
      const float pass = (p >= LEPS && p <= ONE_M_EPS) ? 1.f : 0.f;
      const float gm = c.focal_gamma;
      float eo, en, deo, den;
      if (c.label_smooth > 0.f) {
        const float uo = 1.f - c.label_smooth - cc;
        const float un = c.label_smooth - cc;
        eo = fabsf(uo);
        en = fabsf(un);
        deo = (uo > 0.f) ? -1.f : (uo < 0.f ? 1.f : 0.f);
        den = (un > 0.f) ? -1.f : (un < 0.f ? 1.f : 0.f);
      } else {
        eo = 1.f - cc;
        en = cc;
        deo = -1.f;
        den = 1.f;
      }
      const bool g2 = gm == 2.f;
      const float ao = g2 ? eo * eo : powf(eo, gm), lo_ = logf(1.f - eo);
      const float an_ = g2 ? en * en : powf(en, gm), ln_ = logf(1.f - en);
      const float lo = -obj * ao * lo_;
      const float ln = -noobj * an_ * ln_;
      part[3] += (double)lo;
      part[4] += (double)ln;
      part[0] += (double)c.loss_weight[1] * ((double)lo + (double)c.binary_weight * (double)ln);
      const float dfo = gm * (g2 ? eo : powf(eo, gm - 1.f)) * lo_ - ao / (1.f - eo);
      const float dfn = gm * (g2 ? en : powf(en, gm - 1.f)) * ln_ - an_ / (1.f - en);
      g = c.loss_weight[1] * (-obj * dfo * deo - c.binary_weight * noobj * dfn * den) * pass;
    }
  } else {
    const float tk = tk_cur;
    const float pc = fminf(fmaxf(p, LEPS), ONE_M_EPS);
    const float pass = (p >= LEPS && p <= ONE_M_EPS) ? 1.f : 0.f;
    const float wcls = (VER == 4) ? c.loss_weight[2] : c.loss_weight[3];
    if (VER != 1 && obj == 0.f) {
      g = 0.f;
    } else if (VER == 3 || VER == 4) {
      const float l = -obj * (tk * logf(pc) + (1.f - tk) * logf(1.f - pc));
      part[5] += (double)l;
      part[0] += (double)wcls * (double)l;
      g = -wcls * obj * (tk / pc - (1.f - tk) / (1.f - pc)) * pass;
    } else if (VER == 2) {
      const float l = -obj * (tk * logf(pc));
      part[5] += (double)l;
      part[0] += (double)wcls * (double)l;
      g = -wcls * obj * (tk / pc) * pass;
    } else {
      const float l = -t4 * tk * logf(pc);
      part[5] += (double)l;
      part[0] += (double)wcls * (double)l;
      g = -wcls * t4 * (tk / pc) * pass;
    }
  }
  return g;
}

template <int VER, bool PREF>
__global__ __launch_bounds__(256) void loss_kernel(const LossParams lp, const float* __restrict__ y_true,
                                                   const float* __restrict__ y_pred, float* __restrict__ dpred,
                                                   double* __restrict__ out) {
  const yolo_loss_cfg& c = lp.c;
  const int A = c.A, C = c.C;
  const int TD = 5 + C;
  const int PD = (VER == 1) ? 5 * A + C : A * (5 + C);
  const int lane = threadIdx.x & 63;
  const long long wave0 = ((long long)blockIdx.x * blockDim.x + threadIdx.x) >> 6;
  const long long nwaves = ((long long)gridDim.x * blockDim.x) >> 6;
  const float gw = (float)c.gw, gh = (float)c.gh;
  const double invN = 1.0 / (double)c.N;

  double part[7] = {0, 0, 0, 0, 0, 0, 0};

  float my_anchor = 1.f;
#pragma unroll
  for (int j = 0; j < 32; ++j)
    if (lane == j) my_anchor = c.use_anchors ? c.anchors[j] : 1.f;

  auto chan_of = [&](int idx, int& b, int& k) {
    if (VER == 1) {
      if (idx < 5 * A) {
        b = idx / 5;
        k = idx - b * 5;
      } else {
        b = 0;
        k = 5 + (idx - 5 * A);
      }
    } else {
      b = idx / TD;
      k = idx - b * TD;
    }
  };
  auto cell_head = [&](long long cell, const float (&Tb)[4], const float t4, const float (&Pb)[4], float& iou, float (&dI)[4],
                       int& resp) {
    iou = -1.f;
    float ciou = 0.f;
    dI[0] = dI[1] = dI[2] = dI[3] = 0.f;
    if (lane < A) {
      const IouOut o = iou_dual<VER == 4>(Tb, Pb, gw, gh);
      iou = o.iou.v;
      ciou = o.ciou.v;
      const D4& src = (VER == 4) ? o.ciou : o.iou;
      for (int i = 0; i < 4; ++i) dI[i] = src.d[i];
    }
    resp = 0;
    float best = __shfl(iou, 0, 64);
    for (int b = 1; b < A; ++b) {
      const float ib = __shfl(iou, b, 64);
      if (ib > best) {
        best = ib;
        resp = b;
      }
    }
    if (lp.dec != nullptr) {
      const unsigned long long ign = __ballot(lane < A && iou < c.ignore_thresh);
      const unsigned long long tru = __ballot(lane < A && iou > c.truth_thresh);
      if (lane == 0) {
        lp.dec[cell * 2] = resp;
        lp.dec[cell * 2 + 1] = (int)((unsigned)(ign & 0xffffu) | ((unsigned)(tru & 0xffffu) << 16));
      }
    }
    if (VER == 4 && lane < A) {
      float obj = t4 * (lane == resp ? 1.f : 0.f);
      if (c.truth_thresh < 1.f) obj = obj + ((iou > c.truth_thresh) ? 1.f : 0.f) * (1.f - obj);
      const double box = (double)(obj * (1.f - ciou));
      part[1] += box;
      part[0] += (double)c.loss_weight[0] * box;
    }
  };

  if constexpr (PREF) {
    constexpr int NCK = 4;
    float pn[NCK], tkn[NCK], tbn, pbn[4];
    auto prefetch = [&](long long cell) {
      const float* T = y_true + cell * TD;
      const float* Pc = y_pred + cell * PD;
#pragma unroll
      for (int q = 0; q < NCK; ++q) {
        int idx = q * 64 + lane;
        idx = idx < PD ? idx : PD - 1;
        int b, k;
        chan_of(idx, b, k);
        pn[q] = Pc[idx];
        tkn[q] = T[k >= 5 ? k : 4];
      }
      tbn = T[lane < 5 ? lane : 4];
      const float* P = Pc + (lane < A ? lane : 0) * TD;
#pragma unroll
      for (int j = 0; j < 4; ++j) pbn[j] = P[j];
    };
    long long cell = wave0;
    if (cell < lp.cells) prefetch(cell);
    for (; cell < lp.cells; cell += nwaves) {
      float pc[NCK], tkc[NCK], Pb[4];
#pragma unroll
      for (int q = 0; q < NCK; ++q) {
        pc[q] = pn[q];
        tkc[q] = tkn[q];
      }
#pragma unroll
      for (int j = 0; j < 4; ++j) Pb[j] = pbn[j];
      const float tbc = tbn;
      if (cell + nwaves < lp.cells) prefetch(cell + nwaves);
      float* G = dpred ? dpred + cell * PD : nullptr;
      const float Tb[4] = {__shfl(tbc, 0, 64), __shfl(tbc, 1, 64), __shfl(tbc, 2, 64), __shfl(tbc, 3, 64)};
      const float t4 = __shfl(tbc, 4, 64);
      float iou, dI[4];
      int resp;
      cell_head(cell, Tb, t4, Pb, iou, dI, resp);
#pragma unroll
      for (int q = 0; q < NCK; ++q) {
        const int base = q * 64;
        if (base < PD) {
          const bool active = (base + lane) < PD;
          const int idx = active ? (base + lane) : (PD - 1);
          int b, k;
          chan_of(idx, b, k);
          const float iou_b = __shfl(iou, b, 64);
          const float d0 = __shfl(dI[0], b, 64), d1 = __shfl(dI[1], b, 64);
          const float d2 = __shfl(dI[2], b, 64), d3 = __shfl(dI[3], b, 64);
          const float an = __shfl(my_anchor, (b * 2 + ((k == 3) ? 1 : 0)) & 31, 64);
          const float r_b = (b == resp) ? 1.f : 0.f;
          if (active) {
            const float g = loss_channel<VER>(c, b, k, pc[q], tkc[q], t4, Tb, iou_b, d0, d1, d2, d3, an, 0.f, r_b, part);
            if (G) G[idx] = g * lp.inv_n;
          }
        }
      }
    }
  } else {
  for (long long cell = wave0; cell < lp.cells; cell += nwaves) {
    const float* T = y_true + cell * TD;
    const float* Pc = y_pred + cell * PD;
    float* G = dpred ? dpred + cell * PD : nullptr;

    const float t4 = T[4];
    const float Tb[4] = {T[0], T[1], T[2], T[3]};
    float Pb[4] = {0.f, 0.f, 0.f, 0.f};
    if (lane < A) {
      const float* P = Pc + ((VER == 1) ? lane * 5 : lane * (5 + C));
      for (int j = 0; j < 4; ++j) Pb[j] = P[j];
    }
    float iou, dI[4];
    int resp;
    cell_head(cell, Tb, t4, Pb, iou, dI, resp);

    float p_nxt, tk_nxt;
    {
      const int idx0 = lane < PD ? lane : (PD - 1);
      int b0, k0;
      chan_of(idx0, b0, k0);
      p_nxt = Pc[idx0];
      tk_nxt = T[k0 >= 5 ? k0 : 4];
    }
    for (int base = 0; base < PD; base += 64) {
      const bool active = (base + lane) < PD;
      const int idx = active ? (base + lane) : (PD - 1);
      int b, k;
      chan_of(idx, b, k);
      const float p = p_nxt, tk_cur = tk_nxt;
      if (base + 64 < PD) {
        const int idn = (base + 64 + lane) < PD ? (base + 64 + lane) : (PD - 1);
        int bn, kn;
        chan_of(idn, bn, kn);
        p_nxt = Pc[idn];
        tk_nxt = T[kn >= 5 ? kn : 4];
      }
      const float iou_b = __shfl(iou, b, 64);
      const float d0 = __shfl(dI[0], b, 64), d1 = __shfl(dI[1], b, 64);
      const float d2 = __shfl(dI[2], b, 64), d3 = __shfl(dI[3], b, 64);
      const float an = __shfl(my_anchor, (b * 2 + ((k == 3) ? 1 : 0)) & 31, 64);
      const float cb = (VER == 1) ? Pc[b * 5 + 4] : 0.f;
      const float r_b = (b == resp) ? 1.f : 0.f;
      if (!active) continue;
      const float g = loss_channel<VER>(c, b, k, p, tk_cur, t4, Tb, iou_b, d0, d1, d2, d3, an, cb, r_b, part);
      if (G) G[idx] = g * lp.inv_n;
    }
  }
  }

  __shared__ double red[7][4];
  const int wave = threadIdx.x >> 6;
#pragma unroll
  for (int q = 0; q < 7; ++q) {
    const double s = wave_reduce_sum(part[q]);
    if (lane == 0) red[q][wave] = s;
  }
  __syncthreads();
  if (threadIdx.x < 7) {
    const double s = red[threadIdx.x][0] + red[threadIdx.x][1] + red[threadIdx.x][2] + red[threadIdx.x][3];
    atomicAdd(&out[threadIdx.x], s * invN);
  }
}

template <int VER>
__global__ __launch_bounds__(256) void metrics_kernel(const LossParams lp, const float* __restrict__ y_true,
                                                      const float* __restrict__ y_pred, float recall_thresh,
                                                      double* __restrict__ out) {
  const yolo_loss_cfg& c = lp.c;
  const int A = c.A, C = c.C;
  const int TD = 5 + C;
  const int PD = (VER == 1) ? 5 * A + C : A * (5 + C);
  const int lane = threadIdx.x & 63;
  const long long wave0 = ((long long)blockIdx.x * blockDim.x + threadIdx.x) >> 6;
  const long long nwaves = ((long long)gridDim.x * blockDim.x) >> 6;
  const float gw = (float)c.gw, gh = (float)c.gh;
  double part[5] = {0, 0, 0, 0, 0};

  for (long long cell = wave0; cell < lp.cells; cell += nwaves) {
    const float* T = y_true + cell * TD;
    const float* Pc = y_pred + cell * PD;
    const float t4 = T[4];
    float iou = -FLT_MAX, conf = -FLT_MAX;
    if (lane < A) {
      const float* P = Pc + ((VER == 1) ? lane * 5 : lane * (5 + C));
      const float Tb[4] = {T[0], T[1], T[2], T[3]};
      const float Pb[4] = {P[0], P[1], P[2], P[3]};
      iou = iou_dual<false>(Tb, Pb, gw, gh).iou.v;
      conf = P[4];
    }
    auto wave_argmax = [&](const float* v) -> int {
      float bv = -FLT_MAX;
      int bi = 0x7fffffff;
      for (int k = lane; k < C; k += 64) {
        const float x = v[k];
        if (x > bv) {
          bv = x;
          bi = k;
        }
      }
      for (int o = 32; o > 0; o >>= 1) {
        const float ov = __shfl_xor(bv, o, 64);
        const int oi = __shfl_xor(bi, o, 64);
        if (ov > bv || (ov == bv && oi < bi)) {
          bv = ov;
          bi = oi;
        }
      }
      return bi;
    };
    const int pi_true = wave_argmax(T + 5);
    float max_conf = -FLT_MAX, max_iou = -FLT_MAX, max_rec = -FLT_MAX;
    float eq_sum = 0.f;
    int pi_pred_cell = 0;
    if (VER == 1) pi_pred_cell = wave_argmax(Pc + 5 * A);
    for (int b = 0; b < A; ++b) {
      const float ib = __shfl(iou, b, 64);
      const float cb = __shfl(conf, b, 64);
      const int pi_pred = (VER == 1) ? pi_pred_cell : wave_argmax(Pc + b * TD + 5);
      const float eq = ((pi_pred == pi_true) ? 1.f : 0.f) * t4;
      max_conf = fmaxf(max_conf, cb);
      max_iou = fmaxf(max_iou, ib);
      max_rec = fmaxf(max_rec, ib * eq);
      eq_sum += eq;
    }
    if (lane == 0) {
      const float pred_bin = (max_conf > 0.5f) ? 1.f : 0.f;
      part[0] += (t4 == pred_bin) ? 1.0 : 0.0;
      part[1] += (double)(max_iou * t4);
      part[2] += (double)t4;
      part[3] += (VER == 1) ? (double)(((pi_pred_cell == pi_true) ? 1.f : 0.f) * t4) : (double)eq_sum;
      part[4] += (max_rec >= recall_thresh) ? 1.0 : 0.0;
    }
  }
  __shared__ double red[5][4];
  const int wave = threadIdx.x >> 6;
  if (lane == 0)
    for (int q = 0; q < 5; ++q) red[q][wave] = part[q];
  __syncthreads();
  if (threadIdx.x < 5) {
    const double s = red[threadIdx.x][0] + red[threadIdx.x][1] + red[threadIdx.x][2] + red[threadIdx.x][3];
    atomicAdd(&out[threadIdx.x], s);
  }
  if (blockIdx.x == 0 && threadIdx.x == 5) out[5] = (double)lp.cells;
}

static int validate_cfg(const yolo_loss_cfg* cfg) {
  YOLO_REQUIRE(cfg != nullptr, "loss: null cfg");
  YOLO_REQUIRE(cfg->version >= 1 && cfg->version <= 4, "loss: bad version %d", cfg->version);
  YOLO_REQUIRE(cfg->N > 0 && cfg->gh > 0 && cfg->gw > 0 && cfg->C > 0, "loss: bad shape");
  YOLO_REQUIRE(cfg->A > 0 && cfg->A <= 16, "loss: anchors per cell %d out of range [1,16]", cfg->A);
  return YOLO_OK;
}

}

using namespace yolo;

extern "C" size_t yolo_loss_workspace_bytes(const yolo_loss_cfg* cfg) {
  (void)cfg;
  return 0;
}

extern "C" int yolo_loss_fwd_bwd(const yolo_loss_cfg* cfg, const float* y_true, const float* y_pred, double* loss_out,
                                 float* dpred, float grad_scale, void* workspace, size_t workspace_bytes,
                                 void* stream) {
  if (int rc = validate_cfg(cfg)) return rc;
  YOLO_REQUIRE(y_true && y_pred && loss_out, "loss: null pointer");
  LossParams lp;
  lp.c = *cfg;
  lp.cells = (long long)cfg->N * cfg->gh * cfg->gw;
  lp.inv_n = grad_scale / (float)cfg->N;
  lp.dec = (workspace != nullptr && workspace_bytes >= (size_t)lp.cells * 8 && cfg->A <= 16) ? reinterpret_cast<int*>(workspace)
                                                                                              : nullptr;
  hipStream_t st = as_stream(stream);
  if (hipMemsetAsync(loss_out, 0, 8 * sizeof(double), st) != hipSuccess) {
    set_error("loss: memset failed");
    return YOLO_ERR_LAUNCH;
  }
  long long blocks = (lp.cells + 3) / 4;
  if (blocks > 2048) blocks = 2048;
  dim3 grid((unsigned)blocks), block(256);
  static const bool pref_env = env_int("YOLO_LOSS_PREFETCH", 1) != 0;
  const bool pref = pref_env && !(g_opt[OPT_EXP] & 8) && cfg->version != 1 && cfg->A * (5 + cfg->C) <= 256;
  switch (cfg->version) {
    case 1: hipLaunchKernelGGL((loss_kernel<1, false>), grid, block, 0, st, lp, y_true, y_pred, dpred, loss_out); break;
    case 2:
      if (pref) hipLaunchKernelGGL((loss_kernel<2, true>), grid, block, 0, st, lp, y_true, y_pred, dpred, loss_out);
      else hipLaunchKernelGGL((loss_kernel<2, false>), grid, block, 0, st, lp, y_true, y_pred, dpred, loss_out);
      break;
    case 3:
      if (pref) hipLaunchKernelGGL((loss_kernel<3, true>), grid, block, 0, st, lp, y_true, y_pred, dpred, loss_out);
      else hipLaunchKernelGGL((loss_kernel<3, false>), grid, block, 0, st, lp, y_true, y_pred, dpred, loss_out);
      break;
    default:
      if (pref) hipLaunchKernelGGL((loss_kernel<4, true>), grid, block, 0, st, lp, y_true, y_pred, dpred, loss_out);
      else hipLaunchKernelGGL((loss_kernel<4, false>), grid, block, 0, st, lp, y_true, y_pred, dpred, loss_out);
      break;
  }
  return check_launch("loss_kernel");
}

extern "C" int yolo_metrics(const yolo_loss_cfg* cfg, const float* y_true, const float* y_pred, float recall_thresh,
                            double* out, void* stream) {
  if (int rc = validate_cfg(cfg)) return rc;
  YOLO_REQUIRE(y_true && y_pred && out, "metrics: null pointer");
  LossParams lp;
  lp.c = *cfg;
  lp.cells = (long long)cfg->N * cfg->gh * cfg->gw;
  lp.inv_n = 0.f;
  hipStream_t st = as_stream(stream);
  if (hipMemsetAsync(out, 0, 8 * sizeof(double), st) != hipSuccess) {
    set_error("metrics: memset failed");
    return YOLO_ERR_LAUNCH;
  }
  long long blocks = (lp.cells + 3) / 4;
  if (blocks > 2048) blocks = 2048;
  dim3 grid((unsigned)blocks), block(256);
  switch (cfg->version) {
    case 1: hipLaunchKernelGGL(metrics_kernel<1>, grid, block, 0, st, lp, y_true, y_pred, recall_thresh, out); break;
    case 2: hipLaunchKernelGGL(metrics_kernel<2>, grid, block, 0, st, lp, y_true, y_pred, recall_thresh, out); break;
    case 3: hipLaunchKernelGGL(metrics_kernel<3>, grid, block, 0, st, lp, y_true, y_pred, recall_thresh, out); break;
    default: hipLaunchKernelGGL(metrics_kernel<4>, grid, block, 0, st, lp, y_true, y_pred, recall_thresh, out); break;
  }
  return check_launch("metrics_kernel");
}
```

tf2_yolo_amd/engine.py:

```python
import math

import contextlib

import numpy as np
import torch

from . import ops
from . import plan
from . import tape
from ._lib import ACT_LEAKY, ACT_LINEAR, ACT_MISH, YoloHipError
from .plan import AUX_WORDS, has_filter

ACT_NAMES = {ACT_LINEAR: "linear", ACT_LEAKY: "leaky", ACT_MISH: "mish"}


class ParamSpec:
    __slots__ = ("name", "shape", "offset", "size", "init", "trainable")

    def __init__(self, name, shape, offset, init, trainable):
        self.name, self.shape, self.offset = name, tuple(shape), offset
        self.size = int(np.prod(shape))
        self.init, self.trainable = init, trainable


# ... 179 lines not shown
    def maxpool(self, src, k, name, stride=None, padding="valid"):
        stride = stride or k
        if padding == "same":
            ho, wo = -(-src.h // stride), -(-src.w // stride)
        else:
            ho, wo = (src.h - k) // stride + 1, (src.w - k) // stride + 1
        return self._push(MaxPoolUnit(name, src, k, stride, padding), ho, wo, src.c)

    def space_to_depth(self, src, name):
        return self._push(SpaceToDepthUnit(name, src), src.h // 2, src.w // 2, src.c * 4)

    def head(self, src, A, C, version, anchors, name, level):
        u = HeadUnit(name, src, A, C, version, anchors, level, self.kernel_init)
        out = self._push(u, src.h, src.w, u.cout)
        self.outputs.append(out)
        return out


def count_params(builder):
    train = state = 0
    for u in builder.units:
        if has_filter(u):
            train += u.cout * u.k * u.k * u.src.c + (u.cout if u.bias else 0) + (2 * u.cout if u.bn else 0)
            state += 2 * u.cout if u.bn else 0
    return train, state


def conv_flops_per_image(builder):
    total = 0
    for u in builder.units:
        if has_filter(u):
            total += 2 * u.out.h * u.out.w * u.cout * u.src.c * u.k * u.k
    return total


_EPILOGUES = {ACT_LEAKY: ops.EPI_AFFINE_LEAKY, ACT_MISH: ops.EPI_AFFINE_MISH}


def _epilogue(u):
    return _EPILOGUES.get(u.act, ops.EPI_AFFINE)


class Network:
    def __init__(self, builder, device="cuda", seed=1234, unbiased_moving_var=True):
        if not torch.cuda.is_available():
            raise YoloHipError("tf2_yolo_amd needs a HIP device: there is no CPU fallback")
        self.device = torch.device(device)
        if self.device.index is not None and self.device.index != torch.cuda.current_device():
            raise YoloHipError(f"Network(device={device!r}): the kernels launch on the current device "
                               f"(cuda:{torch.cuda.current_device()}); call torch.cuda.set_device first "
                               "(one process per GPU)")
        self.tensors = builder.tensors
        self.units = builder.units
        self.input = builder.input
        self.outputs = list(builder.outputs)
        self.unbiased_moving_var = unbiased_moving_var
        self._opts = plan.Options.from_env()
        for k, v in vars(self._opts).items():
            setattr(self, "_" + k, v)
        g = self._plan = plan.plan_graph(self.units, self.tensors, self.input, self.outputs, self._opts)
        self._needs_grad, self._n_consumers = g.needs_grad, g.n_consumers
        self._bound_alias, self._up_producer = g.bound_alias, g.up_producer
        self.params = ParamStore()
        self.state = ParamStore()
        self._declare_params()
        rng = np.random.default_rng(seed)
        self.params.materialize(self.device, rng)
        self.state.materialize(self.device, rng)
        self.grads = torch.zeros_like(self.params.data)
        self._init_anchors()
        ops.create_side_streams(self.device)
        ops.ensure_conv_workspace()
        ops.ensure_wgrad_workspace()
        self._alloc_planned_buffers(g)
        self._wT_valid = self._wp_valid = self._wTp_valid = False
        self._jobs_wp = self._jobs_wTp = self._jobs_wT = None
        self._wp_event = self._wT_event = None
        self._infer_graphs = {}
        self._wgrad_stream = None
        self._wgrad_pending = False
        self.batch = None
        self.act = {}
        self.training = False
        self.grad_ready_hook = None
        self.backward_begin_hook = None
        self._infer_scale_valid = False
        self._twords = None
        self._tword_n = {}
        self._xplanes_infer = {}
        for u in self.units:
            u.concat_reads_through = False

    def _declare_params(self):
        for u in self.units:
            if u.kind == "conv":
                u.p_kernel = self.params.add(f"{u.name}_conv/kernel", (u.cout, u.k, u.k, u.src.c), u.kernel_init)
                u.p_bias = self.params.add(f"{u.name}_conv/bias", (u.cout,), init_zeros) if u.bias else None
                if u.bn:
                    u.p_gamma = self.params.add(f"{u.name}_bn/gamma", (u.cout,), init_ones)
                    u.p_beta = self.params.add(f"{u.name}_bn/beta", (u.cout,), init_zeros)
                    u.s_mean = self.state.add(f"{u.name}_bn/moving_mean", (u.cout,), init_zeros)
                    u.s_var = self.state.add(f"{u.name}_bn/moving_variance", (u.cout,), init_ones)
            elif u.kind == "head":
                u.p_kernel = self.params.add(f"{u.name}/kernel", (u.cout, 1, 1, u.src.c), u.kernel_init)
                u.p_bias = self.params.add(f"{u.name}/bias", (u.cout,), init_zeros)

    def _init_anchors(self):
        self._anchors_dev, self._anchor_grad_views = {}, {}
        heads = [u for u in self.units if u.kind == "head" and u.anchors is not None]
        n_anch = sum(2 * len(u.anchors) for u in heads)
        self.anchors_flat = torch.zeros(max(n_anch, 1), device=self.device, dtype=torch.float32)
        self.anchor_grads = torch.zeros_like(self.anchors_flat)
        self.anchors_trainable = False
        off = 0
        for u in heads:
            n = 2 * len(u.anchors)
            self.anchors_flat[off:off + n] = torch.tensor(np.array(u.anchors, dtype=np.float32).reshape(-1))
            self._anchors_dev[u.name] = self.anchors_flat[off:off + n]
            self._anchor_grad_views[u.name] = self.anchor_grads[off:off + n]
            off += n
        self.has_anchors = n_anch > 0

    def _alloc_planned_buffers(self, g):
        dev = self.device
        self._wT = torch.empty(g.wT_total, device=dev, dtype=torch.float32)
        self._bn_f32 = torch.zeros(max(g.bn_f32_total, 1), device=dev, dtype=torch.float32)
        self._bn_f64 = torch.zeros(max(g.bn_f64_total, 1), device=dev, dtype=torch.float64)
        self._bn_stats_total = g.bn_stats_total
        self._wplanes = torch.empty(g.wplanes_total, device=dev, dtype=torch.uint8) if g.wplanes_total else None
        self._aux = torch.zeros(g.aux_total, device=dev, dtype=torch.int32)
        self._tbound = self._aux[g.tbound_off:].view(torch.float32)
        self._tb = [self._tbound[i:i + 1] for i in range(len(self.tensors))]
        self._pred = torch.zeros(g.pred_total, device=dev, dtype=torch.float32)
        for u in self.units:
            a = u.aux_off
            u.bound = self._aux[a:a + 1]
            u.red_bound = self._aux[a + 1:a + 69]
            u.tickets = self._aux[a + 69:a + 69 + ops.BN_FOLD_TICKET_WORDS]
            u.pred = self._pred[u.pred_off:u.pred_off + 2]
            if u.kind == "conv" and u.bn:
                u.amax = self._aux[a + AUX_WORDS:a + AUX_WORDS + u.cout]
            if not has_filter(u):
                continue
            u.wT = self._wT[u.wT_off:u.wT_off + u.cout * u.k * u.k * u.src.c]
            u.wp = self._wplanes[u.wp_off:u.wp_off + u.wp_bytes] if u.planes_fwd else None
            u.wTp = self._wplanes[u.wTp_off:u.wTp_off + u.wTp_bytes] if u.planes_dgrad else None
            if u.cpad:
                u.wTp_pad = self._wplanes[u.wTp_pad_off:u.wTp_pad_off + u.wTp_pad_bytes]
                n = u.cpad * u.src.c
                u.w_pad = torch.zeros(n, device=dev, dtype=torch.float32)
                u.wT_pad = torch.empty(n, device=dev, dtype=torch.float32)
                u.dw_pad = torch.empty(n, device=dev, dtype=torch.float32)

    @property
    def num_params(self):
        return sum(self.params.specs[n].size for n in self.params.order)

    @property
    def num_state(self):
        return sum(self.state.specs[n].size for n in self.state.order)

    def allocate(self, N):
        if self.batch == N:
            return
        worst = max((t.h * t.w * t.c * 4 for t in self.tensors), default=0)
        if worst and N * worst + (1 << 20) >= (1 << 32):
# ... 91 lines not shown
            for u in self._filter_units():
                if u.cpad:
                    self._jobs_wTp.add_split(u.wT_pad, u.wTp_pad, u.src.c, u.cpad)
                elif u.planes_dgrad:
                    self._jobs_wTp.add_split(u.wT, u.wTp, u.src.c, u.k * u.k * u.cout, bound_from=u.wp)
        self._jobs_wTp.run()
        self._wTp_valid = True

    def _refresh_wT(self):
        if self._wT_valid:
            return
        if self._jobs_wT is None:
            self._jobs_wT = ops.BatchJobs("transpose", self.device)
            for u in self._filter_units():
                if u.cpad:
                    self._jobs_wT.add_transpose(u.w_pad, u.wT_pad, u.cpad, 1, u.src.c)
                else:
                    self._jobs_wT.add_transpose(self.params.view(u.p_kernel.name), u.wT, u.cout, u.k * u.k, u.src.c)
        for u in self.units:
            if u.kind == "head" and u.cpad:
                tape.torch_op(lambda u=u: u.w_pad[:u.out.c * u.src.c].copy_(self.params.view(u.p_kernel.name).reshape(-1)))
        self._jobs_wT.run()
        self._wT_valid = True

    def _conv_fwd(self, u, bias, out, stats=None, absmax=None):
        if u.planes_fwd:
            return ops.conv2d_fwd_planes(u.desc, self._xp(u.src), u.wp, bias, out=out, stats=stats, absmax=absmax)
        return ops.conv2d_fwd(u.desc, self.act[u.src.tid], self.params.view(u.p_kernel.name), bias, out=out, stats=stats,
                              absmax=absmax)

    def _tight_bound(self, u):
        m = self._bn_tight
        return m == 1 or (m == 2 and u.k != 1)

    def _bn_bufs(self, u):
        c = u.cout
        b = self._bn_f32[u.bn_f32_off:u.bn_f32_off + 4 * c]
        ns = ops.BN_STAT_SLOTS * 2 * c
        nr = (ops.BN_RED_SLOTS + 1) * 2 * c
        return (b[0:c], b[c:2 * c], b[2 * c:3 * c], b[3 * c:4 * c], self._bn_f64[u.bn_f64_off:u.bn_f64_off + ns],
                self._bn_f64[u.bn_red_off:u.bn_red_off + nr])

    def _fold_infer_scale(self, u, scale, shift):
        if self._infer_scale_valid:
            return False
        ops.bn_fold_inference(u.cout, self.params.view(u.p_gamma.name), self.params.view(u.p_beta.name),
                              self.state.view(u.s_mean.name), self.state.view(u.s_var.name), scale, shift)
        return True

    def infer(self, x):
        if not self._use_infer_graph:
            return self.forward(x, training=False)
        x = x.contiguous()
        N = x.shape[0]
        g = self._infer_graphs.get(N)
        if g is None:
            self.forward(x, training=False)
            static_in = x.clone()
            self.forward(static_in, training=False)
            torch.cuda.synchronize()
            graph = torch.cuda.CUDAGraph()
            with torch.cuda.graph(graph):
                outs = self.forward(static_in, training=False)
            g = self._infer_graphs[N] = (graph, static_in, outs)
        graph, static_in, outs = g
        static_in.copy_(x)
        graph.replay()
        return outs

    def before_param_write(self):
        for ev in (self._wp_event, self._wT_event):
            if ev is not None:
                torch.cuda.current_stream().wait_event(ev)
        self._wp_event = self._wT_event = None

    def mark_params_changed(self):
        self.before_param_write()
        self._infer_graphs = {}
        self._wT_valid = False
        self._wp_valid = False
        self._wTp_valid = False
        self._infer_scale_valid = False

    def forward(self, x, training=False, stop_after=None):
        if x.dtype != torch.float32 or not x.is_cuda:
            raise YoloHipError("forward expects a float32 CUDA tensor")
        x = x.contiguous()
        if tuple(x.shape[1:]) != (self.input.h, self.input.w, self.input.c):
            raise YoloHipError(f"input shape {tuple(x.shape[1:])} != model input "
                               f"{(self.input.h, self.input.w, self.input.c)}")
        self.allocate(x.shape[0])
        self.training = training
        self.act[self.input.tid] = x
        self._xp_valid = set()
        self._tbound_set = set()
        self._tword_n = {}
        self._prepare_filters(training)
        ops.zero_bytes(self._aux)
        if training:
            ops.zero_bytes(self._bn_f64[:self._bn_stats_total])
            self._infer_scale_valid = False
            self._infer_graphs = {}
        prev_name = None
        for u in self.units:
            if stop_after is not None and prev_name == stop_after:
                self.training = False
                return None
            prev_name = u.name
            if self._wp_event is not None and has_filter(u) and u.planes_fwd:
                tape.wait_event(torch.cuda.current_stream(), self._wp_event)
                self._wp_event = None
            fwd = getattr(self, "_fwd_" + u.kind, None)
            if fwd is None:
                raise YoloHipError(f"unknown unit kind {u.kind}")
            fwd(u, training)
        if not training:
            self._infer_scale_valid = True
        return [self.act[t.tid] for t in self.outputs]

    def _prepare_filters(self, training):
        if training and self._overlap_wgrad and self._prep_beside and not (self._wp_valid and self._wT_valid and self._wTp_valid):
            if self._wgrad_stream is None:
                self._wgrad_stream = ops.concurrent_stream("wgrad", device=self.device)
            side = self._wgrad_stream
            tape.wait_stream(side, torch.cuda.current_stream())
            with torch.cuda.stream(side):
                self._refresh_wplanes()
                self._wp_event = tape.record_event(side)
                self._refresh_wT()
                self._refresh_wTplanes()
                self._wT_event = tape.record_event(side)
        else:
            self._refresh_wplanes()

    def _fwd_conv(self, u, training):
        bias = self.params.view(u.p_bias.name) if u.p_bias is not None else None
        if not u.bn:
            self._conv_fwd(u, bias, u.y)
            if u.act != ACT_LINEAR:
                ops.act_fwd(u.y, u.act, out=u.a)
            if u.residual is not None:
                raise YoloHipError("residual without BN is not used by any reference graph")
            return
        scale, shift, smean, sinv, stats, _ = self._bn_bufs(u)
        if training:
            amax = u.amax if self._tight_bound(u) else None
            self._conv_fwd(u, None, u.y, stats, amax)
            ops.bn_finalize(stats, u.y.numel() // u.cout, u.cout, self.params.view(u.p_gamma.name),
                            self.params.view(u.p_beta.name), self.state.view(u.s_mean.name), self.state.view(u.s_var.name),
                            scale, shift, smean, sinv, unbiased=self.unbiased_moving_var, bound=u.bound, absmax=amax,
                            mean_offset=bias)
            if u.pool_fuse is not None:
                return self._fwd_bn_act_pool(u, scale, shift)
        elif self._fuse_infer and (self._fused_infer_unit(u, bias, scale, shift)
                                   or (self._infer_onepass and self._stem_infer_unit(u, bias, scale, shift))):
            return
        else:
            self._conv_fwd(u, bias, u.y, absmax=u.amax)
            self._fold_infer_scale(u, scale, shift)
            ops.bn_infer_bound(u.cout, scale, shift, u.amax, u.bound)
        self._fwd_bn_act(u, training, scale, shift)

    def _fwd_bn_act_pool(self, u, scale, shift):
        pu = u.pool_fuse
        ppl = self._xplanes.get(pu.out.tid) if pu.out.c % 16 == 0 else None
        ops.bn_act_maxpool2x2_fwd(u.y, u.cout, scale, shift, u.act, pu.argmax,
                                  out=pu.buf if (pu.f32_needed or ppl is None) else None, planes=ppl,
                                  bn_bound=u.bound, out_bound=self._tb[pu.out.tid])
        self._tbound_set.add(pu.out.tid)
        if ppl is not None:
            self._xp_valid.add(pu.out.tid)
        pu.fused_this_pass = True

    def _fwd_bn_act(self, u, training, scale, shift):
        res = self.act[u.residual.tid] if u.residual is not None else None
        res_pl = None
        if (res is not None and training and self._res_from_planes and u.cout % 16 == 0
                and u.residual.tid in self._xp_valid and u.residual.tid in self._tbound_set):
            res_pl, res = self._xplanes[u.residual.tid], None
        pl = self._xplanes.get(u.out.tid) if u.cout % 16 == 0 else None
        if u.residual is not None and u.residual.tid not in self._tbound_set:
            pl = None
        else:
            self._tbound_set.add(u.out.tid)
        ops.bn_act_fwd(u.y, u.cout, scale, shift, u.act, res, out=u.a, planes=pl,
                       want_out=not (training and pl is not None and not u.a_needed), bn_bound=u.bound,
                       residual_bound=self._tb_float(u.residual.tid) if res is not None else None,
                       out_bound=self._tb[u.out.tid], residual_planes=res_pl)
        if pl is not None:
            self._xp_valid.add(u.out.tid)

    def _fwd_head(self, u, training):
        bias, anchors = self.params.view(u.p_bias.name), self._anchors_dev.get(u.name)
        if not training and self._infer_small_fuse and self._fuse_infer and u.planes_fwd:
            ops.conv2d_fwd_head_unit(u.desc, self._xp(u.src), u.wp, bias, u.A, u.C, u.version, anchors, u.t, u.yact)
            return
        self._conv_fwd(u, bias, u.t)
        ops.head_act_fwd(u.t, u.A, u.C, u.version, anchors, out=u.yact)

    def _fwd_upsample(self, u, training):
        if not training and self._infer_small_fuse and self._concat_planes and u.out.tid in self._up_producer:
            u.concat_reads_through = True
            return
        ops.upsample2x_fwd(self.act[u.src.tid], u.buf, u.out.c, 0)

    def _fwd_concat(self, u, training):
        pl = self._xplanes.get(u.out.tid) if self._concat_planes else None
        slots = [self._bound_alias.get(s.tid, s.tid) for s in u.srcs]
        ups = [self._up_producer.get(s.tid) for s in u.srcs]
        ups = [p if (p is not None and p.concat_reads_through) else None for p in ups]
        for p in ups:
            if p is not None:
                p.concat_reads_through = False
        rows, chans = self.batch * u.out.h * u.out.w, [s.c for s in u.srcs]
        dst32 = u.buf if u.f32_needed else None
        if (pl is not None and len(u.srcs) <= 4 and all(sl in self._tbound_set for sl in slots)
                and all(s.c % 8 == 0 for s in u.srcs)):
            if any(p is not None for p in ups):
                ops.split_planes_concat_ex([self.act[p.src.tid] if p is not None else self.act[s.tid]
                                            for s, p in zip(u.srcs, ups)], chans, [self._tb_words(sl) for sl in slots],
                                           rows, pl, upsample=[p is not None for p in ups], hw=(u.out.h, u.out.w),
                                           dst32=dst32, out_bound=self._tb[u.out.tid])
            else:
                ops.split_planes_concat([self.act[s.tid] for s in u.srcs], chans, [self._tb_float(sl) for sl in slots],
                                        rows, pl, dst32=dst32, out_bound=self._tb[u.out.tid])
            self._xp_valid.add(u.out.tid)
            self._tbound_set.add(u.out.tid)
            return
        for p in ups:
            if p is not None:
                ops.upsample2x_fwd(self.act[p.src.tid], p.buf, p.out.c, 0)
        off = 0
        for s in u.srcs:
            ops.copy_channels_in(self.act[s.tid], s.c, u.buf, u.out.c, off)
            off += s.c

    def _fwd_maxpool(self, u, training):
        if getattr(u, "fused_this_pass", False):
            u.fused_this_pass = False
            return
        ops.maxpool_fwd(self.act[u.src.tid], u.k, u.stride, u.pad_t, u.pad_l, u.out.h, u.out.w, u.buf,
                        u.out.c, 0, u.argmax if training else None)

    def _fwd_space_to_depth(self, u, training):
        ops.space_to_depth2_fwd(self.act[u.src.tid], u.buf, u.out.c, 0)

    def _stem_infer_unit(self, u, bias, scale, shift):
        pl = self._xplanes.get(u.out.tid)
        if u.residual is not None or pl is None or u.src.tid != self.input.tid or not ops.stem_infer_supported(u.desc):
            return False
        xin, w = self.act[u.src.tid], self.params.view(u.p_kernel.name)
        if self._fold_infer_scale(u, scale, shift):
            if getattr(u, "stem_wt", None) is None:
                u.stem_wt = torch.empty(28 * 32, device=self.device, dtype=torch.float32)
            ops.stem_filter_prep(w, bias, u.stem_wt)
            ops.zero_bytes(u.pred)
            ops.conv_pred_bound(w, u.cout, 27, scale, shift, bias, u.pred)
        row = self._tb_row(self.input.tid)
        n_in = ops.absmax_words(xin, row)
        nw = ops.stem_fwd_infer_unit(u.desc, xin, u.stem_wt, _epilogue(u), scale, shift, u.pred, row[:n_in],
                                     u.a if u.a_needed else None, pl, self._tb_row(u.out.tid))
        self._tword_n[u.out.tid] = nw
        self._tbound_set.add(u.out.tid)
        self._xp_valid.add(u.out.tid)
        return True

    def _fused_infer_unit(self, u, bias, scale, shift):
        if not u.planes_fwd or u.cout % 16 != 0:
            return False
        pl = self._xplanes.get(u.out.tid)
        own_planes = pl is not None
        if pl is None and self._infer_small_fuse and self._infer_onepass:
            rows = self.batch * u.out.h * u.out.w
            if rows <= 4096:
                pl = self._xplanes_infer.get(u.out.tid)
                if pl is None:
                    pl = self._xplanes_infer[u.out.tid] = torch.zeros(ops.planes_bytes(rows, u.cout), device=self.device,
                                                                     dtype=torch.uint8)
        if pl is None or (u.residual is not None and u.residual.tid not in self._tbound_set):
            return False
        self._fold_infer_scale(u, scale, shift)
# ... 18 lines not shown
        ops.conv2d_fwd_planes_epi(u.desc, self._xp(u.src), u.wp, bias, _epilogue(u), scale, shift, residual=res, out=u.a,
                                  absmax=u.amax)
        ops.split_planes_absmax(u.a, self.batch * u.out.h * u.out.w, u.cout, u.amax, pl,
                                extra_bound=self._tb_float(u.residual.tid) if u.residual is not None else None,
                                out_bound=self._tb[u.out.tid])
        self._tbound_set.add(u.out.tid)
        self._xp_valid.add(u.out.tid)
        return True

    def _stem_fused_bwd(self, u):
        return (self._stem_fused and not (u.planes_wgrad or u.planes_dgrad) and not self._needs_grad[u.src.tid]
                and ops.stem_bn_bwd_supported(u.desc))

    def _takes_grad_slice(self, u):
        return u.kind == "conv" and u.bn and u.residual is None and u.cout % 8 == 0 and not self._stem_fused_bwd(u)

    def _add_grad(self, grads, t, buf):
        if not self._needs_grad[t.tid]:
            return
        cur = grads.get(t.tid)
        if cur is None:
            grads[t.tid] = buf
        else:
            ops.axpy(cur, buf)

    def _grad_into(self, grads, t):
        cur = grads.get(t.tid)
        if cur is not None:
            return cur, True
        cur = grads[t.tid] = torch.empty((self.batch, t.h, t.w, t.c), device=self.device, dtype=torch.float32)
        return cur, False

    def _gview(self, spec):
        return self.grads[spec.offset:spec.offset + spec.size]

    def backward(self, douts):
        if not self.training:
            raise YoloHipError("backward() requires a preceding forward(training=True)")
        if self.backward_begin_hook is not None:
            tape.host_call(self.backward_begin_hook)
        if self._wT_event is not None:
            tape.wait_event(torch.cuda.current_stream(), self._wT_event)
            self._wT_event = None
        self._refresh_wT()
        self._refresh_wTplanes()
        for u in self.units:
            if getattr(u, "bnred", None) is not None:
                u.bnred_done = False
        grads = {t.tid: g for t, g in zip(self.outputs, douts)}
        for u in reversed(self.units):
            dout = grads.pop(u.out.tid, None)
            if dout is None:
                continue
            if isinstance(dout, ops.ChannelSlice) and not self._takes_grad_slice(u):
                dout = dout.dense((self.batch, u.out.h, u.out.w, u.out.c))
            getattr(self, "_bwd_" + u.kind)(u, dout, grads)
            if self.grad_ready_hook is not None and has_filter(u):
                tape.host_call(lambda u=u: self.grad_ready_hook(u))
        self._join_wgrad()

    def _bwd_conv(self, u, dout, grads):
        if u.bn:
            scale, shift, smean, sinv, _, red = self._bn_bufs(u)
            if u.residual is not None:
                self._add_grad(grads, u.residual, dout)
            if self._stem_fused_bwd(u):
                ops.stem_bn_bwd_wgrad(u.desc, self.act[u.src.tid], u.y, dout, scale, shift, smean, sinv, u.act, red,
                                      self._gview(u.p_gamma), self._gview(u.p_beta), self._gview(u.p_kernel),
                                      fused=self._take_fused(u, dout))
                return
            need_f32 = (not u.planes_wgrad) or (self._needs_grad[u.src.tid] and not u.planes_dgrad)
            dyp = self._next_dyp_buffer(u) if (u.planes_wgrad or u.planes_dgrad) else None
            dy = ops.bn_act_bwd(u.y, dout, u.cout, self.params.view(u.p_gamma.name), scale, shift, smean,
                                sinv, u.act, red, self._gview(u.p_gamma), self._gview(u.p_beta),
                                planes=dyp, want_dx=need_f32, bound_aux=u.red_bound, fused=self._take_fused(u, dout),
                                tickets=u.tickets if self._bn_fold else None)
        else:
            dy = ops.act_bwd(u.y, dout, u.act) if u.act != ACT_LINEAR else dout
            dyp = self._dyp(u, dy)
        dbias = self._gview(u.p_bias) if (u.p_bias is not None and not u.bn) else None
        self._filter_and_data_grad(u, dy, dyp, dbias, grads)

    def _bwd_head(self, u, dout, grads):
        dt = ops.head_act_bwd(u.yact, dout, u.A, u.C, u.version, self._anchors_dev.get(u.name),
                              danchors=self._anchor_grad_views.get(u.name) if self.anchors_trainable else None)
        if not u.cpad:
            return self._filter_and_data_grad(u, dt, self._dyp(u, dt), self._gview(u.p_bias), grads)
        rows = self.batch * u.out.h * u.out.w
        dtp = ops.split_planes_padded(dt, rows, u.out.c, out=self._next_dyp_buffer(u))
        with self._beside_backward(dt):
            ops.zero_bytes(u.dw_pad)
            ops.conv2d_wgrad_planes(u.desc_pad, self._xplanes[u.src.tid], dtp, u.dw_pad)
            ops.axpy(self._gview(u.p_kernel), u.dw_pad[:u.out.c * u.src.c])
            ops.conv2d_wgrad_bias(dt, rows, u.out.c, self._gview(u.p_bias))
        if self._needs_grad[u.src.tid]:
            had = grads.get(u.src.tid)
            b = self._bnred_of(u, had)
            cur, acc = self._grad_into(grads, u.src)
            ops.conv2d_dgrad_planes(u.desc_pad, dtp, u.wTp_pad, dx=cur, accumulate=acc, bnred=b)

    def _filter_and_data_grad(self, u, dy, dyp, dbias, grads):
        with self._beside_backward(dy):
            if u.planes_wgrad:
                ops.conv2d_wgrad_planes(u.desc, self._xplanes[u.src.tid], dyp, self._gview(u.p_kernel), dy=dy, dbias=dbias)
            else:
                ops.conv2d_wgrad(u.desc, self.act[u.src.tid], dy, self._gview(u.p_kernel), dbias)
        if not self._needs_grad[u.src.tid]:
            return
        b = self._bnred_of(u, grads.get(u.src.tid)) if u.planes_dgrad else None
        cur, acc = self._grad_into(grads, u.src)
        if u.planes_dgrad:
            ops.conv2d_dgrad_planes(u.desc, dyp, u.wTp, dx=cur, accumulate=acc, bnred=b)
        else:
            ops.conv2d_dgrad(u.desc, dy, u.wT, dx=cur, accumulate=acc)

    def _bwd_upsample(self, u, dout, grads):
        if self._needs_grad[u.src.tid]:
            cur, acc = self._grad_into(grads, u.src)
            ops.upsample2x_bwd(dout, u.out.c, 0, cur, accumulate=acc)

    def _bwd_concat(self, u, dout, grads):
        off = 0
        for s in u.srcs:
            if not self._needs_grad[s.tid]:
                pass
            elif (s.tid not in grads and self._concat_grad_slices and self._n_consumers.get(s.tid, 0) == 1
                    and s.producer is not None and self._takes_grad_slice(s.producer)
                    and s.c % 8 == 0 and off % 4 == 0 and u.out.c % 4 == 0):
                grads[s.tid] = ops.ChannelSlice(dout, u.out.c, off, s.c)
            else:
                cur, acc = self._grad_into(grads, s)
                ops.copy_channels_out(dout, u.out.c, off, cur, s.c, accumulate=acc)
            off += s.c

    def _bwd_maxpool(self, u, dout, grads):
        if not self._needs_grad[u.src.tid]:
            return
        N, had = self.batch, grads.get(u.src.tid)
        tiles = (u.k == 2 and u.stride == 2 and u.pad_t == 0 and u.pad_l == 0 and u.src.h == 2 * u.out.h
                 and u.src.w == 2 * u.out.w and u.out.c % 4 == 0 and torch.is_tensor(dout) and dout.is_contiguous()
                 and (had is None or torch.is_tensor(had)))
        cur, acc = self._grad_into(grads, u.src)
        if tiles:
            ops.maxpool2x2_bwd(dout, N, u.out.h, u.out.w, u.out.c, u.argmax, cur, acc)
            return
        if not acc:
            ops.zero_bytes(cur)
        if u.stride == 1 and (u.out.h, u.out.w) == (u.src.h, u.src.w):
            ops.maxpool_bwd_same(dout, N, u.out.h, u.out.w, u.out.c, u.out.c, 0, u.argmax, u.k, u.pad_t, u.pad_l, cur)
        else:
            ops.maxpool_bwd(dout, N, u.out.h, u.out.w, u.out.c, u.out.c, 0, u.argmax, cur)

    def _bwd_space_to_depth(self, u, dout, grads):
        if self._needs_grad[u.src.tid]:
            cur, acc = self._grad_into(grads, u.src)
            ops.space_to_depth2_bwd(dout, u.out.c, 0, cur, accumulate=acc)

    def _next_dyp_buffer(self, u=None):
        if u is not None and u.name in self._dyp_own:
            self._dyp_cur_own = True
            return self._dyp_own[u.name]
        self._dyp_cur_own = False
        self._dyp_idx ^= 1
        ev = self._dyp_events[self._dyp_idx]
        if ev is not None:
            tape.wait_event(torch.cuda.current_stream(), ev)
            self._dyp_events[self._dyp_idx] = None
        if self._dyplanes2[self._dyp_idx] is None and self._dyp_shared_bytes:
            self._dyplanes2[self._dyp_idx] = torch.empty(self._dyp_shared_bytes, device=self.device, dtype=torch.uint8)
        return self._dyplanes2[self._dyp_idx]

    @contextlib.contextmanager
# ... 72 lines not shown
```

tf2_yolo_amd/model.py:

```python
import time

import numpy as np
import torch

from . import dp as dp_mod
from . import optimizers as opt_mod
from ._lib import YoloHipError
from .engine import Network


def _to_input(x):
    if torch.is_tensor(x):
        return x.to(device="cuda", dtype=torch.float32).contiguous()
    return torch.from_numpy(np.ascontiguousarray(np.asarray(x, dtype=np.float32))).cuda()


class LayerView:

    def __init__(self, model, name, getter, setter, trainable=True):
        self.model, self.name, self._get, self._set, self.trainable = model, name, getter, setter, trainable

    def get_weights(self):
        return self._get()

# ... 228 lines not shown
        self.optimizer = optimizer
        self.optimizer.bind(self.net)
        nout = len(self.net.outputs)
        self.loss = list(loss) if isinstance(loss, (list, tuple)) else [loss] * nout
        if len(self.loss) != nout:
            raise ValueError(f"need {nout} losses, got {len(self.loss)}")
        if metrics is None:
            metrics = [[] for _ in range(nout)]
        elif nout == 1 and (not metrics or not isinstance(metrics[0], (list, tuple))):
            metrics = [list(metrics)]
        self.metrics = [list(m) for m in metrics]
        self._loss_bufs = [torch.zeros(8, device="cuda", dtype=torch.float64) for _ in range(nout)]
        self._dpred = None
        self._drop_step_graphs()

    def enable_data_parallel(self, process_group=None, bucket_bytes=48 << 20):
        segs, units = dp_mod.network_segments(self.net)
        self._reducer = dp_mod.GradReducer(self.net.grads, segs, process_group, bucket_bytes)
        index = {id(u): i for i, u in enumerate(units)}
        self._dp_unit_index = index
        self._drop_step_graphs()
        self.net.grad_ready_hook = lambda u: self._reducer.segment_done(index[id(u)])
        self.net.backward_begin_hook = self._reducer.backward_begin
        net = self.net
        self._reducer.extra_streams = lambda: [net._wgrad_stream] if net._wgrad_stream is not None else []
        dp_mod.broadcast_parameters([self.net.params.data, self.net.state.data], 0, process_group)
        self.net.mark_params_changed()

    def _labels(self, y):
        ys = [y] if not isinstance(y, (list, tuple)) else list(y)
        out = []
        for a in ys:
            if torch.is_tensor(a):
                out.append(a.to(device="cuda", dtype=torch.float32).contiguous())
            else:
                out.append(torch.from_numpy(np.ascontiguousarray(np.asarray(a, dtype=np.float32))).cuda())
        return out

    def _drop_step_graphs(self):
        self._step_graphs = None
        self._eager_steps = {}

    def _captured_step(self, x, y_list):
        import os
        mode = os.environ.get("YOLO_STEP_MODE", "tape")
        if os.environ.get("YOLO_STEP_GRAPH", "1") == "0" or mode == "eager" or getattr(self, "_graphs_failed", False):
            return None
        if not getattr(self.optimizer, "capturable", False):
            return None
        if self.net.grad_ready_hook is not None and self._reducer is None:
            return None
        from .capture import StepGraphs, StepTape
        self.net.allocate(x.shape[0])
        key = StepGraphs.key_of(self, x)
        g = self._step_graphs
        if g is not None and g.key == key:
            return g.replay(x, y_list)
        n = self._eager_steps.get(key, 0)
        if os.environ.get("YOLO_STEP_DEBUG"):
            import sys
            print(f"[step] mode {mode} eager steps so far {n} key {key} known {list(self._eager_steps)}", file=sys.stderr)
        if n < 2 or self._dpred is None:
            self._eager_steps = {key: n + 1}
            self._step_graphs = None
            return None
        try:
            if mode == "graph":
                self._step_graphs = StepGraphs(self, x, y_list)
                return self._step_graphs.replay(x, y_list)
            self._step_graphs = StepTape(self, x, y_list)
            return self._loss_bufs
        except Exception as e:
            import sys
            import traceback
            print(f"[tf2_yolo_amd] step recording ({mode}) failed ({e!r}); training continues with eager launches\n"
                  + "".join(traceback.format_exc().splitlines(True)[-12:]), file=sys.stderr)
            self._graphs_failed = True
            self._step_graphs = None
            if mode != "graph":
                from . import ops as _ops
                _ops.zero_bytes(self.net.grads)
            return None

    def train_step_device(self, x, y_list, with_metrics=False):
        if self.optimizer is None:
            raise YoloHipError("compile() the model before training")
        from . import ops as _ops
        if not with_metrics and _ops.TIMER is None:
            bufs = self._captured_step(x, y_list)
            if bufs is not None:
                return bufs, None
        outs = self.net.forward(x, training=True)
        if self._dpred is None or self._dpred[0].shape != outs[0].shape:
            self._dpred = [torch.empty_like(o) for o in outs]
        for i, (o, yt) in enumerate(zip(outs, y_list)):
            self.loss[i].fwd_bwd(yt, o, grad_scale=1.0, dpred=self._dpred[i], loss_out=self._loss_bufs[i])
        mvals = None
        if with_metrics:
            mvals = [[m(yt, o) for m in ms] for ms, o, yt in zip(self.metrics, outs, y_list)]
        self.net.backward(self._dpred)
        if self._reducer is not None and self.net.anchors_trainable and self._reducer.world > 1:
            import torch.distributed as dist
            dist.all_reduce(self.net.anchor_grads, group=self._reducer.pg)
        scale = self._reducer.finish() if self._reducer is not None else 1.0
        self.optimizer.step(grad_scale=scale)
        return self._loss_bufs, mvals

    def train_on_batch(self, x, y, return_dict=False, **_):
        bufs, mvals = self.train_step_device(_to_input(x), self._labels(y), with_metrics=bool(self.metrics))
        losses = [float(b[0].item()) for b in bufs]
        total = sum(losses)
        flat = [float(v.item()) for ms in (mvals or []) for v in ms]
        res = [total] + (losses if len(losses) > 1 else []) + flat
        return res if len(res) > 1 else res[0]

    def test_on_batch(self, x, y):
        outs = self.net.forward(_to_input(x), training=False)
        ys = self._labels(y)
        losses = [float(l(yt, o).item()) for l, o, yt in zip(self.loss, outs, ys)]
        mvals = [float(m(yt, o).item()) for ms, o, yt in zip(self.metrics, outs, ys) for m in ms]
        return [sum(losses)] + (losses if len(losses) > 1 else []) + mvals

    def _iter_batches(self, x, y, batch_size, shuffle, rng):
        if y is None:
            order = np.arange(len(x))
            for i in order:
                yield x[int(i)]
            if hasattr(x, "on_epoch_end"):
                x.on_epoch_end()
            return
        n = len(x)
        order = rng.permutation(n) if shuffle else np.arange(n)
        ys = y if isinstance(y, (list, tuple)) else [y]
        for i in range(0, n, batch_size):
            sel = order[i:i + batch_size]
            yb = [a[sel] for a in ys]
            yield x[sel], (yb if isinstance(y, (list, tuple)) else yb[0])

    def _host_source(self, x, y, batch_size, shuffle, rng):
        if y is None:
            def batches():
                for i in range(len(x)):
                    yield x[int(i)]
                if hasattr(x, "on_epoch_end"):
                    x.on_epoch_end()
            return ("batches", batches())
        ys = list(y) if isinstance(y, (list, tuple)) else [y]
        if any(torch.is_tensor(a) and a.is_cuda for a in [x] + ys):
            return None
        n = len(x)
        order = rng.permutation(n) if shuffle else np.arange(n)
        return ("arrays", [x] + ys, order, batch_size)

    def fit(self, x=None, y=None, batch_size=None, epochs=1, verbose=1, validation_data=None, shuffle=True,
            initial_epoch=0, callbacks=None, **_):
        import os
        from .feeder import FeederBuffers, HostFeeder
        batch_size = batch_size or 32
        rng = np.random.default_rng(0)
        hist = {"loss": []}
        pipelined = os.environ.get("YOLO_FIT_PIPELINE", "1") != "0"
        cbs = list(callbacks or [])

        def _cb(hook, *args):
            for c in cbs:
                f = getattr(c, hook, None)
                if f is not None:
                    f(*args)
        for c in cbs:
            if hasattr(c, "set_model"):
                c.set_model(self)
        self.stop_training = False
        _cb("on_train_begin", {})
        for ep in range(initial_epoch, epochs):
            t0 = time.time()
            _cb("on_epoch_begin", ep, {})
            tot, nb = 0.0, 0
            src = self._host_source(x, y, batch_size, shuffle, rng) if pipelined else None
            if src is not None:
# ... 45 lines not shown
```

tf2_yolo_amd/ops.py:

```python
import ctypes
from ctypes import byref, c_void_p

import torch

from . import _lib
from . import tape as _tape
from ._lib import ConvDesc, LossCfg, YoloHipError, check

BN_EPS = 1e-3
BN_MOMENTUM = 0.99
BN_STAT_SLOTS = 64
BN_RED_SLOTS = 512
SPLIT_BATCH_UNITS = 4


class KernelTimer:

    def __init__(self):
        self.pending = []

    def bracket(self, name, flops, launches, fn, layer=None):
        s, e = torch.cuda.Event(enable_timing=True), torch.cuda.Event(enable_timing=True)
        s.record()
        fn()
# ... 232 lines not shown
        if t is None:
            continue
        if not (t.is_cuda and t.dtype == torch.float32 and t.is_contiguous()):
            raise YoloHipError("expected a contiguous float32 CUDA tensor, got "
                               f"{t.dtype} {t.device} contiguous={t.is_contiguous()}")


def same_pad(size, k, s):
    out = -(-size // s)
    total = max((out - 1) * s + k - size, 0)
    return out, total // 2


def conv_desc(x_shape, cout, kh, kw, stride, padding):
    n, h, w, cin = x_shape
    if padding == "same":
        ho, pt = same_pad(h, kh, stride)
        wo, pl = same_pad(w, kw, stride)
    elif padding == "valid":
        ho, wo, pt, pl = (h - kh) // stride + 1, (w - kw) // stride + 1, 0, 0
    elif padding == "darknet_s2":
        ho, wo, pt, pl = (h + 1 - kh) // stride + 1, (w + 1 - kw) // stride + 1, 1, 1
    else:
        raise ValueError(f"bad padding {padding}")
    return ConvDesc(n, h, w, cin, cout, kh, kw, ho, wo, stride, stride, pt, pl)


def conv2d_fwd(d, x, w, bias=None, out=None, stats=None, absmax=None):
    _chk_f32(x, w, bias)
    if out is None:
        out = torch.empty((d.N, d.Ho, d.Wo, d.Cout), device=x.device, dtype=torch.float32)
    if x.numel() != d.N * d.H * d.W * d.Cin or w.numel() != d.Cout * d.kh * d.kw * d.Cin:
        raise YoloHipError("conv2d_fwd: tensor sizes do not match the descriptor")
    if out.numel() != d.N * d.Ho * d.Wo * d.Cout:
        raise YoloHipError("conv2d_fwd: output size does not match the descriptor")
    if stats is not None and stats.numel() != BN_STAT_SLOTS * 2 * d.Cout:
        raise YoloHipError("conv2d_fwd: stats must hold BN_STAT_SLOTS x 2 x Cout doubles")
    def run():
        check(_lib.load().yolo_conv2d_fwd_absmax(byref(d), _p(x), _p(w), _p(bias), _p(out), _p(stats), _p(absmax),
                                                 _stream()), "yolo_conv2d_fwd")
    if TIMER is not None:
        stem = (CONV_MODE == "split" and _os.environ.get("YOLO_STEM_DIRECT", "1") != "0" and d.Cin == 3 and d.Cout == 32
                and d.kh == 3 and d.kw == 3 and d.sh == 1 and d.sw == 1 and d.Ho == d.H and d.Wo == d.W
                and d.N * d.H * d.W >= (1 << 20))
        name = "stem_conv3x3_kernel" if stem else _gather_variant(d.Cout, d.Cin % 32 != 0, d.N * d.Ho * d.Wo)
        TIMER.bracket(name, _conv_flops(d), 1, run)
    else:
        run()
    return out


def planes_bytes(rows, c):
    n = int(_lib.load().yolo_planes_bytes(int(rows), int(c)))
    if n == 0:
        raise YoloHipError(f"planes: unsupported shape rows={rows} C={c} (C must be a multiple of 16)")
    return n


def split_planes(x, rows, c, out=None):
    _chk_f32(x)
    if x.numel() != rows * c:
        raise YoloHipError("split_planes: tensor size does not match rows x C")
    n = planes_bytes(rows, c)
    if out is None:
        out = torch.empty(n, device=x.device, dtype=torch.uint8)
    elif out.numel() < n or out.dtype != torch.uint8:
        raise YoloHipError("split_planes: output buffer too small")
    check(_lib.load().yolo_split_planes(_p(x), int(rows), int(c), _p(out), _stream()), "yolo_split_planes")
    return out


def split_planes_padded(x, rows, c_src, out=None):
    _chk_f32(x)
    c = (c_src + 15) // 16 * 16
    if x.numel() != rows * c_src:
        raise YoloHipError("split_planes_padded: tensor size does not match rows x C_src")
    n = planes_bytes(rows, c)
    if out is None:
        out = torch.empty(n, device=x.device, dtype=torch.uint8)
    elif out.numel() < n or out.dtype != torch.uint8:
        raise YoloHipError("split_planes_padded: output buffer too small")
    check(_lib.load().yolo_split_planes_padded(_p(x), int(rows), int(c_src), int(c), _p(out), _stream()),
          "yolo_split_planes_padded")
    return out


class BatchJobs:

    def __init__(self, kind, device):
        self.kind, self.device = kind, device
        self.rows, self.blocks, self.table = [], 0, None

    def add_split(self, src, dst, rows, c, bound_from=None):
        nb = -(-((rows + 15) // 16 + 1) // SPLIT_BATCH_UNITS) * -(-c // 128)
        donor = 0 if bound_from is None else bound_from.data_ptr() + bound_from.numel() - 256
        self.rows.append([src.data_ptr(), dst.data_ptr(), rows, c, donor, self.blocks])
        self.blocks += nb

    def add_transpose(self, src, dst, cout, taps, cin):
        nb = -(-cin // 32) * -(-cout // 32) * taps
        self.rows.append([src.data_ptr(), dst.data_ptr(), cout, taps, cin, self.blocks])
        self.blocks += nb

    def run(self):
        if not self.rows:
            return
        if self.table is None:
            self.table = torch.tensor(self.rows, dtype=torch.int64).to(self.device)
        fn = _lib.load().yolo_split_planes_batch if self.kind == "split" else _lib.load().yolo_filter_transpose_batch
        check(fn(_p(self.table), len(self.rows), self.blocks, _stream()), "yolo_%s_batch" % self.kind)


def conv2d_fwd_planes(d, xp, wp, bias=None, out=None, stats=None, absmax=None):
    _chk_f32(bias)
    if out is None:
        out = torch.empty((d.N, d.Ho, d.Wo, d.Cout), device=xp.device, dtype=torch.float32)
    if xp.numel() < planes_bytes(d.N * d.H * d.W, d.Cin) or wp.numel() < planes_bytes(d.Cout, d.kh * d.kw * d.Cin):
        raise YoloHipError("conv2d_fwd_planes: planes buffers do not match the descriptor")
    if out.numel() != d.N * d.Ho * d.Wo * d.Cout:
        raise YoloHipError("conv2d_fwd_planes: output size does not match the descriptor")
    if stats is not None and stats.numel() != BN_STAT_SLOTS * 2 * d.Cout:
        raise YoloHipError("conv2d_fwd_planes: stats must hold BN_STAT_SLOTS x 2 x Cout doubles")
    def run():
        check(_lib.load().yolo_conv2d_fwd_planes(byref(d), _p(xp), _p(wp), _p(bias), _p(out), _p(stats), _p(absmax),
                                                 _stream()), "yolo_conv2d_fwd_planes")
    if TIMER is not None:
        TIMER.bracket(_planes_variant(d.Cout, _win_key(d, d.H, d.W, d.Cin), d.kh * d.kw == 1), _conv_flops(d), 1, run,
                      _layer_key(d, "fwd"))
    else:
        run()
    return out


EPI_NONE, EPI_AFFINE, EPI_AFFINE_LEAKY, EPI_AFFINE_MISH = 0, 1, 2, 3


def conv2d_fwd_planes_epi(d, xp, wp, bias, epilogue, scale, shift, residual=None, out=None, absmax=None):
    _chk_f32(bias, scale, shift, residual)
    if out is None:
        out = torch.empty((d.N, d.Ho, d.Wo, d.Cout), device=xp.device, dtype=torch.float32)
    if xp.numel() < planes_bytes(d.N * d.H * d.W, d.Cin) or wp.numel() < planes_bytes(d.Cout, d.kh * d.kw * d.Cin):
        raise YoloHipError("conv2d_fwd_planes_epi: planes buffers do not match the descriptor")
    if out.numel() != d.N * d.Ho * d.Wo * d.Cout or (residual is not None and residual.numel() != out.numel()):
        raise YoloHipError("conv2d_fwd_planes_epi: output / residual size does not match the descriptor")
    def run():
        check(_lib.load().yolo_conv2d_fwd_planes_epi(byref(d), _p(xp), _p(wp), _p(bias), int(epilogue), _p(scale), _p(shift),
                                                     _p(residual), _p(out), _p(absmax), _stream()),
              "yolo_conv2d_fwd_planes_epi")
    if TIMER is not None:
        TIMER.bracket(_planes_variant(d.Cout, _win_key(d, d.H, d.W, d.Cin), d.kh * d.kw == 1), _conv_flops(d), 1, run,
                      _layer_key(d, "fwd"))
    else:
        run()
    return out


def conv_pred_bound(w, cout, kdim, scale, shift, bias, pred2):
    _chk_f32(w, scale, shift, bias, pred2)
    if w.numel() != cout * kdim or pred2.numel() != 2:
        raise YoloHipError("conv_pred_bound: w must hold Cout x kdim floats, pred2 two")
    check(_lib.load().yolo_conv_pred_bound(_p(w), int(cout), int(kdim), _p(scale), _p(shift), _p(bias), _p(pred2), _stream()),
          "yolo_conv_pred_bound")


INFER_BOUND_WORDS = 4096

# ... 480 lines not shown
def maxpool_bwd_same(dy, N, H, W, C, Cy, c_off, argmax, k, pad_t, pad_l, dx):
    check(_lib.load().yolo_maxpool_bwd_same(_p(dy), N, H, W, C, Cy, c_off, _p(argmax), int(k), int(pad_t), int(pad_l), _p(dx),
                                            _stream()), "yolo_maxpool_bwd_same")


def space_to_depth2_fwd(x, y, Cy, c_off):
    n, h, w, c = x.shape
    check(_lib.load().yolo_space_to_depth2_fwd(_p(x), n, h, w, c, _p(y), Cy, c_off, _stream()),
          "yolo_space_to_depth2_fwd")


def space_to_depth2_bwd(dy, Cy, c_off, dx, accumulate=False):
    n, h, w, c = dx.shape
    check(_lib.load().yolo_space_to_depth2_bwd(_p(dy), n, h, w, c, Cy, c_off, _p(dx), int(bool(accumulate)),
                                               _stream()), "yolo_space_to_depth2_bwd")


def head_act_fwd(t, A, C, version, anchors_dev, out=None):
    if out is None:
        out = torch.empty_like(t)
    D = (5 * A + C) if version == 1 else A * (5 + C)
    P = t.numel() // D
    check(_lib.load().yolo_head_act_fwd(_p(t), P, A, C, version, _p(anchors_dev), _p(out), _stream()),
          "yolo_head_act_fwd")
    return out


def head_act_bwd(y, dy, A, C, version, anchors_dev, dt=None, danchors=None):
    if dt is None:
        dt = torch.empty_like(y)
    D = (5 * A + C) if version == 1 else A * (5 + C)
    P = y.numel() // D
    check(_lib.load().yolo_head_act_bwd(_p(y), _p(dy), P, A, C, version, _p(anchors_dev), _p(dt), _p(danchors),
                                        _stream()), "yolo_head_act_bwd")
    return dt


def make_loss_cfg(version, N, gh, gw, A, C, anchors=None, binary_weight=1.0, loss_weight=(1, 1, 1, 1),
                  ignore_thresh=0.6, use_focal_loss=False, focal_gamma=2.0, use_scale=True, wh_reg_weight=0.01,
                  truth_thresh=1.0, label_smooth=0.0):
    cfg = LossCfg()
    cfg.version, cfg.N, cfg.gh, cfg.gw, cfg.A, cfg.C = version, N, gh, gw, A, C
    if anchors is not None:
        flat = [float(v) for pair in anchors for v in pair]
        if len(flat) != 2 * A or len(flat) > 32:
            raise ValueError(f"need {A} (w,h) anchors, at most 16; got {len(flat) // 2}")
        for i, v in enumerate(flat):
            cfg.anchors[i] = v
        cfg.use_anchors = 1
    else:
        cfg.use_anchors = 0
    cfg.binary_weight = float(binary_weight)
    lw = list(loss_weight) + [0.0] * (4 - len(loss_weight))
    for i in range(4):
        cfg.loss_weight[i] = float(lw[i])
    cfg.ignore_thresh = float(ignore_thresh)
    cfg.use_focal_loss = int(bool(use_focal_loss))
    cfg.focal_gamma = float(focal_gamma)
    cfg.use_scale = int(bool(use_scale))
    cfg.wh_reg_weight = float(wh_reg_weight)
    cfg.truth_thresh = float(truth_thresh)
    cfg.label_smooth = float(label_smooth)
    return cfg


def loss_fwd_bwd(cfg, y_true, y_pred, loss_out=None, dpred=None, grad_scale=1.0, want_grad=True, decisions=None):
    _chk_f32(y_true, y_pred, dpred)
    cells = cfg.N * cfg.gh * cfg.gw
    pd = (5 * cfg.A + cfg.C) if cfg.version == 1 else cfg.A * (5 + cfg.C)
    if y_true.numel() != cells * (5 + cfg.C) or y_pred.numel() != cells * pd:
        raise YoloHipError(f"loss: tensor sizes do not match cfg (cells={cells}, C={cfg.C}, A={cfg.A})")
    if loss_out is None:
        loss_out = torch.empty(8, device=y_pred.device, dtype=torch.float64)
    if want_grad and dpred is None:
        dpred = torch.empty_like(y_pred)
    if decisions is not None and (decisions.dtype != torch.int32 or decisions.numel() < 2 * cells or not decisions.is_cuda):
        raise YoloHipError("loss: decisions must be an int32 CUDA tensor with 2 entries per cell")
    check(_lib.load().yolo_loss_fwd_bwd(byref(cfg), _p(y_true), _p(y_pred), _p(loss_out),
                                        _p(dpred if want_grad else None), float(grad_scale), _p(decisions),
                                        0 if decisions is None else decisions.numel() * 4, _stream()), "yolo_loss_fwd_bwd")
    return loss_out, dpred


def metrics(cfg, y_true, y_pred, recall_thresh=0.5, out=None):
    _chk_f32(y_true, y_pred)
    if out is None:
        out = torch.empty(8, device=y_pred.device, dtype=torch.float64)
    check(_lib.load().yolo_metrics(byref(cfg), _p(y_true), _p(y_pred), float(recall_thresh), _p(out), _stream()),
          "yolo_metrics")
    return out


def encode_labels(boxes, cls, first, n_images, img_hw, grid_shape, class_num):
    if boxes.dtype != torch.float64 or cls.dtype != torch.int32 or first.dtype != torch.int32:
        raise YoloHipError("encode_labels: boxes float64, cls / first int32")
    gh, gw = grid_shape
    l64 = torch.empty((n_images, gh, gw, 5 + class_num), device=boxes.device, dtype=torch.float64)
    l32 = torch.empty((n_images, gh, gw, 5 + class_num), device=boxes.device, dtype=torch.float32)
    check(_lib.load().yolo_encode_labels(_p(boxes.contiguous()), _p(cls.contiguous()), _p(first.contiguous()), n_images,
                                         float(img_hw[0]), float(img_hw[1]), gh, gw, class_num, _p(l64), _p(l32),
                                         _stream()), "yolo_encode_labels")
    return l64, l32


def down2xlabel(label64):
    if label64.dtype != torch.float64 or not label64.is_cuda or not label64.is_contiguous():
        raise YoloHipError("down2xlabel: contiguous float64 CUDA tensor expected")
    n, gh, gw, ch = label64.shape
    o64 = torch.empty((n, gh // 2, gw // 2, ch), device=label64.device, dtype=torch.float64)
    o32 = torch.empty((n, gh // 2, gw // 2, ch), device=label64.device, dtype=torch.float32)
    check(_lib.load().yolo_down2xlabel(_p(label64), n, gh, gw, ch, _p(o64), _p(o32), _stream()), "yolo_down2xlabel")
    return o64, o32


def adam_step(p, g, m, v, lr, step, beta1=0.9, beta2=0.999, eps=1e-7, grad_scale=1.0, zero_grad=True):
    check(_lib.load().yolo_adam_step(_p(p), _p(g), _p(m), _p(v), p.numel(), lr, beta1, beta2, eps, int(step),
                                     float(grad_scale), int(bool(zero_grad)), _stream()), "yolo_adam_step")


def adam_lr_t(lr, step, beta1=0.9, beta2=0.999):
    return float(_lib.load().yolo_adam_lr_t(float(lr), float(beta1), float(beta2), int(step)))


def adam_step_dev(p, g, m, v, hyper, zero_grad=True):
    check(_lib.load().yolo_adam_step_dev(_p(p), _p(g), _p(m), _p(v), p.numel(), _p(hyper), int(zero_grad), _stream()),
          "yolo_adam_step_dev")


def sgd_step(p, g, lr, grad_scale=1.0, zero_grad=True):
    check(_lib.load().yolo_sgd_step(_p(p), _p(g), p.numel(), lr, float(grad_scale), int(bool(zero_grad)), _stream()),
          "yolo_sgd_step")


OPT_CHUNK = 8192
CLIP_NONE, CLIP_NORM, CLIP_GLOBAL, CLIP_VALUE = 0, 1, 2, 3
OPT_HYPER = 8


def build_chunk_table(variables, chunk=OPT_CHUNK):
    import numpy as np
    if chunk <= 0 or chunk % 4:
        raise ValueError("chunk must be a positive multiple of 4 floats")
    offs, lens, owner, first = [], [], [], [0]
    end = 0
    for v, (off, size) in enumerate(variables):
        off, size = int(off), int(size)
        if off < end or size < 0:
            raise ValueError(f"variable {v} (offset {off}, size {size}) overlaps the one before it")
        end = off + size
        for o in range(off, end, chunk):
            offs.append(o)
            lens.append(min(chunk, end - o))
            owner.append(v)
        first.append(len(offs))
    return (np.asarray(offs, dtype=np.int64), np.asarray(lens, dtype=np.int32), np.asarray(owner, dtype=np.int32),
            np.asarray(first, dtype=np.int32))


class ChunkTable:

    def __init__(self, variables, chunk=OPT_CHUNK, device="cuda"):
        off, ln, var, first = build_chunk_table(variables, chunk)
        if len(off) == 0:
            raise YoloHipError("ChunkTable: no elements")
        self.n_chunks, self.n_vars = len(off), len(first) - 1
        self.extent = int(off[-1] + ln[-1])
# ... 209 lines not shown
```

tf2_yolo_amd/plan.py:

```python
import os
from types import SimpleNamespace

from . import ops

AUX_WORDS = 112


class Options:

    @classmethod
    def from_env(cls, env=None):
        env = os.environ if env is None else env
        o = cls()

        def on(name):
            return env.get(name, "1") != "0"
        o.overlap_wgrad = on("YOLO_BWD_OVERLAP")
        o.prep_beside = on("YOLO_PREP_OVERLAP")
        o.stem_fused = on("YOLO_STEM_FUSED_BWD")
        o.bn_tight = int(env.get("YOLO_BN_TIGHT_BOUND", "0"))
        o.res_from_planes = on("YOLO_RES_PLANES")
        o.use_infer_graph = on("YOLO_INFER_GRAPH")
        o.fuse_infer = on("YOLO_INFER_FUSE")
        o.concat_grad_slices = on("YOLO_CONCAT_GRAD_SLICE")
        o.dyp_per_layer = on("YOLO_DYP_PER_LAYER")
        o.bn_fold = env.get("YOLO_BN_FOLD", "0") == "1"
        o.bn_fused_reduce = env.get("YOLO_BN_FUSED_REDUCE", "0")
        o.head_pad = on("YOLO_HEAD_PAD")
        o.pool_fuse = on("YOLO_POOL_FUSE")
        o.concat_planes = on("YOLO_CONCAT_PLANES")
        o.infer_onepass = on("YOLO_INFER_ONEPASS")
        o.infer_small_fuse = on("YOLO_INFER_SMALL_FUSE")
        o.dgrad_classes = on("YOLO_DGRAD_CLASSES")
        return o


def has_filter(u):
    return u.kind in ("conv", "head")


def reads_as_planes(c, t):
    return has_filter(c) and c.src.tid == t.tid and c.residual is not t and c.planes_fwd and c.planes_wgrad


def _fp32_read(t, g, also=lambda c: False):
    cs = g.consumers.get(t.tid, [])
    return t.tid in g.out_tids or not cs or any(not (reads_as_planes(c, t) or also(c)) for c in cs)


def plan_graph(units, tensors, input, outputs, opts):
    g = SimpleNamespace(out_tids={t.tid for t in outputs})
    g.needs_grad = {input.tid: False}
    for u in units:
        g.needs_grad[u.out.tid] = has_filter(u) or any(g.needs_grad[t.tid] for t in u.inputs)
    g.consumers, g.n_consumers = {}, {}
    for u in units:
        for t in u.inputs:
            g.consumers.setdefault(t.tid, []).append(u)
            g.n_consumers[t.tid] = g.n_consumers.get(t.tid, 0) + 1
    for t in outputs:
        g.n_consumers[t.tid] = g.n_consumers.get(t.tid, 0) + 1
    _plan_param_buffers(g, units)
    _plan_fused_reduce(g, units, tensors, opts)
    _plan_filter_planes(g, units, opts)
    _plan_fp32_copies(g, units, opts)
    _plan_bounds(g, units, tensors)
    return g


def _plan_param_buffers(g, units):
    wT = f32 = f64 = 0
    for u in units:
        if u.kind == "conv" and u.bn:
            u.bn_f32_off = f32
            f32 += 4 * u.cout
            u.bn_f64_off = f64
            f64 += ops.BN_STAT_SLOTS * 2 * u.cout
        if has_filter(u):
            u.wT_off = wT
            wT += u.cout * u.k * u.k * u.src.c
    g.bn_stats_total = f64
    for u in units:
        if u.kind == "conv" and u.bn:
            u.bn_red_off = f64
            f64 += (ops.BN_RED_SLOTS + 1) * 2 * u.cout
    g.wT_total, g.bn_f32_total, g.bn_f64_total = wT, f32, f64


def _plan_fused_reduce(g, units, tensors, opts):
    last = {}
    for u in reversed(units):
        u.bnred_for = None
        if u.kind == "conv" and u.bn and u.residual is not None and g.needs_grad[u.residual.tid]:
            last[u.residual.tid] = ("add", u)
        if has_filter(u):
            if g.needs_grad[u.src.tid]:
                last[u.src.tid] = ("dgrad", u)
        else:
            for t in u.inputs:
                if g.needs_grad[t.tid]:
                    last[t.tid] = ("other", u)
    mode = opts.bn_fused_reduce
    if mode == "0":
        return
    for tid, (how, w) in last.items():
        p = tensors[tid].producer
        if how != "dgrad":
            continue
        one_launch = w.stride == 1 or (w.stride == 2 and w.k == 3 and opts.dgrad_classes)
        if not (one_launch and p is not None and p.kind == "conv" and p.bn and p.cout % 4 == 0):
            continue
        if w.kind == "head":
            cls = "h"
        elif w.stride == 2:
            cls = "s"
        elif w.k == 1:
            cls = "p"
        else:
            cls = "w"
        w.bnred_class = cls
        if mode == "1" or cls in mode or (cls == "w" and "t" in mode):
            w.bnred_for = p


def _plan_filter_planes(g, units, opts):
    total = 0

    def region(nbytes):
        nonlocal total
        off = total
        total += (nbytes + 255) // 256 * 256
        return off, nbytes
    for u in filter(has_filter, units):
        cin, taps = u.src.c, u.k * u.k
        u.planes_fwd = ops.planes_fwd_ok(cin, u.cout)
        u.planes_dgrad = ops.planes_dgrad_ok(cin, u.cout) and g.needs_grad[u.src.tid]
        u.planes_wgrad = u.planes_fwd and ops.planes_wgrad_ok(cin, u.cout, taps, u.stride)
        u.wp_off = u.wTp_off = -1
        u.cpad = 0
        if u.kind == "head" and u.cout % 16 != 0 and not u.planes_dgrad and opts.head_pad:
            cp = (u.cout + 15) // 16 * 16
            if u.planes_fwd and ops.planes_wgrad_ok(cin, cp, 1) and ops.planes_dgrad_ok(cin, cp):
                u.cpad = cp
                u.wTp_pad_off, u.wTp_pad_bytes = region(ops.planes_bytes(cin, cp))
        if u.planes_fwd:
            u.wp_off, u.wp_bytes = region(ops.planes_bytes(u.cout, taps * cin))
        if u.planes_dgrad:
            u.wTp_off, u.wTp_bytes = region(ops.planes_bytes(cin, taps * u.cout))
    g.wplanes_total = total


def _plan_fp32_copies(g, units, opts):
    for u in units:
        u.pool_fuse = None
        if u.kind != "conv":
            continue
        def adds_from_planes(c, t=u.out):
            return (opts.res_from_planes and c.kind == "conv" and c.bn and c.residual is t and c.src.tid != t.tid
                    and c.cout % 16 == 0)
        cs = g.consumers.get(u.out.tid, [])
        has_planes_src = any(has_filter(c) and c.src.tid == u.out.tid and c.planes_fwd for c in cs)
        u.a_needed = u.cout % 16 != 0 or not has_planes_src or _fp32_read(u.out, g, also=adds_from_planes)
        if not opts.pool_fuse or not u.bn or u.residual is not None or u.out.tid in g.out_tids:
            continue
        if len(cs) != 1 or cs[0].kind != "maxpool":
            continue
        p = cs[0]
        if (p.k == 2 and p.stride == 2 and u.out.h % 2 == 0 and u.out.w % 2 == 0 and p.out.h * 2 == u.out.h
                and p.out.w * 2 == u.out.w and u.cout % 8 == 0 and p.padding in ("same", "valid")):
            p.f32_needed = p.out.c % 16 != 0 or _fp32_read(p.out, g)
            u.pool_fuse = p
    g.bound_alias, g.up_producer = {}, {}
    for u in units:
        if u.kind in ("upsample", "maxpool", "space_to_depth"):
            g.bound_alias[u.out.tid] = g.bound_alias.get(u.src.tid, u.src.tid)
        elif u.kind == "concat":
            u.f32_needed = _fp32_read(u.out, g)
        if u.kind == "upsample" and g.n_consumers.get(u.out.tid, 0) == 1 and u.out.tid not in g.out_tids:
            cs = g.consumers.get(u.out.tid, [])
            if (len(cs) == 1 and cs[0].kind == "concat" and u.out.h == 2 * u.src.h and u.out.w == 2 * u.src.w
                    and u.out.c == u.src.c):
                g.up_producer[u.out.tid] = u


def _plan_bounds(g, units, tensors):
    off = 0
    for i, u in enumerate(units):
        u.aux_off = off
        off += AUX_WORDS
        if u.kind == "conv" and u.bn:
            off += (u.cout + 7) // 8 * 8
        u.pred_off = 2 * i
    g.tbound_off = max(off, 1)
    g.aux_total = g.tbound_off + max(len(tensors), 1) + 1
    g.pred_total = 2 * max(len(units), 1)


def plan_batch(units, N, opts):
    b = SimpleNamespace(desc={}, desc_pad={}, pool_pad={}, xplanes_bytes={}, dyp_own_bytes={}, dyp_shared_bytes=0,
                        bnred_cap={})
    for u in units:
        if u.kind == "maxpool":
            same = u.padding == "same"
            b.pool_pad[u.name] = (ops.same_pad(u.src.h, u.k, u.stride)[1] if same else 0,
                                  ops.same_pad(u.src.w, u.k, u.stride)[1] if same else 0)
        if not has_filter(u):
            continue
        shape = (N, u.src.h, u.src.w, u.src.c)
        b.desc[u.name] = ops.conv_desc(shape, u.cout, u.k, u.k, u.stride, u.padding)
        if u.planes_fwd and u.src.tid not in b.xplanes_bytes:
            b.xplanes_bytes[u.src.tid] = ops.planes_bytes(N * u.src.h * u.src.w, u.src.c)
        if u.cpad:
            b.desc_pad[u.name] = ops.conv_desc(shape, u.cpad, 1, 1, 1, "same")
        elif not (u.planes_dgrad or u.planes_wgrad):
            continue
        nb = ops.planes_bytes(N * u.out.h * u.out.w, u.cpad or u.cout)
        b.dyp_shared_bytes = max(b.dyp_shared_bytes, nb)
        if opts.dyp_per_layer:
            b.dyp_own_bytes[u.name] = nb
    for w in units:
        p = w.bnred_for
        if p is None or not (w.planes_dgrad or w.cpad):
            continue
        if getattr(w, "bnred_class", "") == "w" and opts.bn_fused_reduce != "1":
            small = -(-N * w.src.h * w.src.w // 128) * -(-w.src.c // 128) <= 256
            if ("t" if small else "w") not in opts.bn_fused_reduce:
                continue
        cap = ops.bnred_slots_cap(b.desc[w.name])
        if cap > 0:
            b.bnred_cap[p.name] = cap
    return b
```

Baseline: 1095.

## Fuse YOLO head activation and its backward into the loss kernel

Adds a loss kernel that reads the raw head logits, applies the sigmoid/exp anchor activation inline, and writes the gradient with respect to the logits directly, so the separate head activation backward kernel is skipped. The same kernel reduces the absolute maximum of the gradient into the header of the padded gradient planes, which lets the plane split skip its own memset and amax pass. The path is enabled by default through a planning check and falls back when metrics are requested, anchors are trainable, or the configuration does not match. It trades a heavier loss kernel (more registers, exp per channel) for fewer launches and fewer full passes over the head gradients.

```diff
diff --git a/include/yolo_hip.h b/include/yolo_hip.h
--- a/include/yolo_hip.h
+++ b/include/yolo_hip.h
@@ -62,6 +62,7 @@
 size_t yolo_planes_bytes(long long rows, int C);
 int yolo_split_planes(const float* x, long long rows, int C, void* planes, void* stream);
 int yolo_split_planes_padded(const float* x, long long rows, int C_src, int C, void* planes, void* stream);
+int yolo_split_planes_padded_bounded(const float* x, long long rows, int C_src, int C, void* planes, void* stream);
 
 int yolo_split_planes_batch(const void* jobs, int njobs, long long total_blocks, void* stream);
 int yolo_filter_transpose_batch(const void* jobs, int njobs, long long total_blocks, void* stream);
@@ -231,6 +232,9 @@
 int yolo_loss_fwd_bwd(const yolo_loss_cfg* cfg, const float* y_true, const float* y_pred,
                       double* loss_out, float* dpred, float grad_scale,
                       void* workspace, size_t workspace_bytes, void* stream);
+int yolo_loss_head_fwd_bwd(const yolo_loss_cfg* cfg, const float* y_true, const float* t, const float* head_anchors,
+                           double* loss_out, float* dt, float grad_scale, void* dy_planes,
+                           void* workspace, size_t workspace_bytes, void* stream);
 
 int yolo_metrics(const yolo_loss_cfg* cfg, const float* y_true, const float* y_pred,
                  float recall_thresh, double* out, void* stream);
diff --git a/tf2_yolo_amd/_lib.py b/tf2_yolo_amd/_lib.py
--- a/tf2_yolo_amd/_lib.py
+++ b/tf2_yolo_amd/_lib.py
@@ -51,6 +51,7 @@
     "yolo_planes_bytes": (c_size_t, [_LL, c_int]),
     "yolo_split_planes": (c_int, [_P, _LL, c_int, _P, _P]),
     "yolo_split_planes_padded": (c_int, [_P, _LL, c_int, c_int, _P, _P]),
+    "yolo_split_planes_padded_bounded": (c_int, [_P, _LL, c_int, c_int, _P, _P]),
     "yolo_split_planes_batch": (c_int, [_P, c_int, _LL, _P]),
     "yolo_filter_transpose_batch": (c_int, [_P, c_int, _LL, _P]),
     "yolo_conv2d_fwd_planes": (c_int, [POINTER(ConvDesc), _P, _P, _P, _P, _P, _P, _P]),
@@ -118,6 +119,7 @@
     "yolo_head_act_bwd": (c_int, [_P, _P, _LL, c_int, c_int, c_int, _P, _P, _P, _P]),
     "yolo_loss_workspace_bytes": (c_size_t, [POINTER(LossCfg)]),
     "yolo_loss_fwd_bwd": (c_int, [POINTER(LossCfg), _P, _P, _P, _P, c_float, _P, c_size_t, _P]),
+    "yolo_loss_head_fwd_bwd": (c_int, [POINTER(LossCfg), _P, _P, _P, _P, _P, c_float, _P, _P, c_size_t, _P]),
     "yolo_metrics": (c_int, [POINTER(LossCfg), _P, _P, c_float, _P, _P]),
     "yolo_adam_step": (c_int, [_P, _P, _P, _P, _LL, c_float, c_float, c_float, c_float, c_int, c_float, c_int, _P]),
     "yolo_adam_lr_t": (c_float, [c_float, c_float, c_float, c_int]),
diff --git a/tf2_yolo_amd/capture.py b/tf2_yolo_amd/capture.py
--- a/tf2_yolo_amd/capture.py
+++ b/tf2_yolo_amd/capture.py
@@ -79,9 +79,7 @@
         try:
             with torch.cuda.stream(stream):
                 begin()
-                outs = net.forward(self.x, training=True)
-                for i, (o, yt) in enumerate(zip(outs, self.ys)):
-                    model.loss[i].fwd_bwd(yt, o, grad_scale=1.0, dpred=model._dpred[i], loss_out=model._loss_bufs[i])
+                model._forward_and_losses(self.x, self.ys)
                 net.backward(model._dpred)
                 net._dyp_events = [None, None]
                 if red is not None:
@@ -149,9 +147,7 @@
         opt.refresh_hyper(grad_scale=(1.0 / red.world) if red is not None else 1.0)
         tape_mod.ACTIVE = self.tape
         try:
-            outs = net.forward(self.x, training=True)
-            for i, (o, yt) in enumerate(zip(outs, self.ys)):
-                model.loss[i].fwd_bwd(yt, o, grad_scale=1.0, dpred=model._dpred[i], loss_out=model._loss_bufs[i])
+            model._forward_and_losses(self.x, self.ys)
             net.backward(model._dpred)
             if red is not None:
                 if net.anchors_trainable and red.world > 1:
diff --git a/tf2_yolo_amd/csrc/conv.hip b/tf2_yolo_amd/csrc/conv.hip
--- a/tf2_yolo_amd/csrc/conv.hip
+++ b/tf2_yolo_amd/csrc/conv.hip
@@ -1041,6 +1041,11 @@
   return launch_split_planes_padded(x, rows, C_src, C, planes, as_stream(stream));
 }
 
+extern "C" int yolo_split_planes_padded_bounded(const float* x, long long rows, int C_src, int C, void* planes, void* stream) {
+  YOLO_REQUIRE(x && planes, "split_planes_padded_bounded: null pointer");
+  return launch_split_planes_padded(x, rows, C_src, C, planes, as_stream(stream), true);
+}
+
 struct BnRedArgs {
   const float* y;
   const float* scale;
diff --git a/tf2_yolo_amd/csrc/conv_args.hpp b/tf2_yolo_amd/csrc/conv_args.hpp
--- a/tf2_yolo_amd/csrc/conv_args.hpp
+++ b/tf2_yolo_amd/csrc/conv_args.hpp
@@ -115,7 +115,7 @@
 int launch_split_planes_concat(const float* const* xs, const int* Cs, const float* const* bounds, int nsrc, long long rows,
                                void* planes, float* dst32, float* out_bound, hipStream_t st,
                                const int* bound_words = nullptr, const int* upsample = nullptr, int H = 0, int W = 0);
-int launch_split_planes_padded(const float* x, long long rows, int Csrc, int C, void* planes, hipStream_t st);
+int launch_split_planes_padded(const float* x, long long rows, int Csrc, int C, void* planes, hipStream_t st, bool bounded = false);
 int launch_split_planes_batch(const void* jobs, int njobs, long long total_blocks, hipStream_t st);
 int launch_filter_transpose_batch(const void* jobs, int njobs, long long total_blocks, hipStream_t st);
 int launch_gather_planes(GatherConvArgs& a, hipStream_t st);
diff --git a/tf2_yolo_amd/csrc/conv_planes.hip b/tf2_yolo_amd/csrc/conv_planes.hip
--- a/tf2_yolo_amd/csrc/conv_planes.hip
+++ b/tf2_yolo_amd/csrc/conv_planes.hip
@@ -785,7 +785,7 @@
   return check_launch("filter_transpose_batch_kernel");
 }
 
-int launch_split_planes_padded(const float* x, long long rows, int Csrc, int C, void* planes, hipStream_t st) {
+int launch_split_planes_padded(const float* x, long long rows, int Csrc, int C, void* planes, hipStream_t st, bool bounded) {
   if (C % 16 != 0 || rows <= 0 || Csrc <= 0 || Csrc > C || C - Csrc >= 16) {
     set_error("split_planes_padded: need 0 < Csrc <= C < Csrc + 16, C %% 16 == 0, rows > 0");
     return YOLO_ERR_INVALID_ARG;
@@ -798,14 +798,16 @@
   }
   unsigned char* out = reinterpret_cast<unsigned char*>(planes);
   unsigned* header = reinterpret_cast<unsigned*>(out + planes_body_bytes(rows, C));
-  if (hipMemsetAsync(header, 0, 16, st) != hipSuccess) {
-    set_error("split_planes_padded: hipMemsetAsync failed");
-    return YOLO_ERR_LAUNCH;
-  }
-  const long long n = rows * Csrc, n4 = n / 4;
-  if (n4 > 0) hipLaunchKernelGGL(planes_amax_kernel, dim3(stream_grid(n4, 256)), dim3(256), 0, st, x, n4, header);
-  if (n > 4 * n4)
-    hipLaunchKernelGGL(planes_amax_scalar_kernel, dim3(1), dim3(256), 0, st, x + 4 * n4, n - 4 * n4, header);
+  if (!bounded) {
+    if (hipMemsetAsync(header, 0, 16, st) != hipSuccess) {
+      set_error("split_planes_padded: hipMemsetAsync failed");
+      return YOLO_ERR_LAUNCH;
+    }
+    const long long n = rows * Csrc, n4 = n / 4;
+    if (n4 > 0) hipLaunchKernelGGL(planes_amax_kernel, dim3(stream_grid(n4, 256)), dim3(256), 0, st, x, n4, header);
+    if (n > 4 * n4)
+      hipLaunchKernelGGL(planes_amax_scalar_kernel, dim3(1), dim3(256), 0, st, x + 4 * n4, n - 4 * n4, header);
+  }
   hipLaunchKernelGGL(split_planes_padded_kernel, dim3((unsigned)blocks), dim3(256), 0, st, x, rows, Csrc, C, out,
                      rows_padded);
   return check_launch("split_planes_padded_kernel");
diff --git a/tf2_yolo_amd/csrc/loss.hip b/tf2_yolo_amd/csrc/loss.hip
--- a/tf2_yolo_amd/csrc/loss.hip
+++ b/tf2_yolo_amd/csrc/loss.hip
@@ -1,5 +1,6 @@
 #include "common.hpp"
 #include "conv_args.hpp"
+#include "planes.hpp"
 #include <cfloat>
 #include <cstdlib>
 
@@ -89,6 +90,20 @@
     o.ciou = o.iou - rho2 / c2 - alpha * v;
   }
   return o;
+}
+
+__device__ __forceinline__ float head_activate(const float v, const bool wh, const float anchor) {
+#pragma clang fp contract(off)
+  const float e = expf(wh ? v : -v);
+  const float y_wh = e * anchor;
+  const float y_sig = 1.f / (1.f + e);
+  return wh ? y_wh : y_sig;
+}
+__device__ __forceinline__ float head_act_grad(const float gs, const float y, const bool wh) {
+#pragma clang fp contract(off)
+  const float gy = gs * y;
+  const float gyy = gy * (1.f - y);
+  return wh ? gy : gyy;
 }
 
 struct LossParams {
@@ -252,10 +267,12 @@
   return g;
 }
 
-template <int VER, bool PREF>
-__global__ __launch_bounds__(256) void loss_kernel(const LossParams lp, const float* __restrict__ y_true,
-                                                   const float* __restrict__ y_pred, float* __restrict__ dpred,
-                                                   double* __restrict__ out) {
+template <int VER, bool PREF, bool HEAD>
+__device__ __forceinline__ void loss_body(const LossParams& lp, const float* __restrict__ y_true,
+                                          const float* __restrict__ y_pred, float* __restrict__ dpred,
+                                          double* __restrict__ out, const float* __restrict__ head_anchors,
+                                          unsigned* __restrict__ bound) {
+  static_assert(!HEAD || (PREF && (VER == 3 || VER == 4)), "the logits form exists for the cell-ahead loader of v3 / v4");
   const yolo_loss_cfg& c = lp.c;
   const int A = c.A, C = c.C;
   const int TD = 5 + C;
@@ -272,6 +289,12 @@
 #pragma unroll
   for (int j = 0; j < 32; ++j)
     if (lane == j) my_anchor = c.use_anchors ? c.anchors[j] : 1.f;
+
+  float head_anchor = 1.f;
+  float amax = 0.f;
+  if constexpr (HEAD) {
+    if (lane < 2 * A) head_anchor = head_anchors[lane];
+  }
 
   auto chan_of = [&](int idx, int& b, int& k) {
     if (VER == 1) {
@@ -358,6 +381,23 @@
       for (int j = 0; j < 4; ++j) Pb[j] = pbn[j];
       const float tbc = tbn;
       if (cell + nwaves < lp.cells) prefetch(cell + nwaves);
+      if constexpr (HEAD) {
+#pragma unroll
+        for (int q = 0; q < NCK; ++q) {
+          int idx = q * 64 + lane;
+          idx = idx < PD ? idx : PD - 1;
+          int b, k;
+          chan_of(idx, b, k);
+          const bool wh = k == 2 || k == 3;
+          pc[q] = head_activate(pc[q], wh, __shfl(head_anchor, (b * 2 + ((k == 3) ? 1 : 0)) & 31, 64));
+        }
+        const int ab = lane < A ? lane : 0;
+        const float aw = __shfl(head_anchor, (ab * 2) & 31, 64), ah = __shfl(head_anchor, (ab * 2 + 1) & 31, 64);
+        Pb[0] = head_activate(Pb[0], false, 1.f);
+        Pb[1] = head_activate(Pb[1], false, 1.f);
+        Pb[2] = head_activate(Pb[2], true, aw);
+        Pb[3] = head_activate(Pb[3], true, ah);
+      }
       float* G = dpred ? dpred + cell * PD : nullptr;
       const float Tb[4] = {__shfl(tbc, 0, 64), __shfl(tbc, 1, 64), __shfl(tbc, 2, 64), __shfl(tbc, 3, 64)};
       const float t4 = __shfl(tbc, 4, 64);
@@ -379,7 +419,13 @@
           const float r_b = (b == resp) ? 1.f : 0.f;
           if (active) {
             const float g = loss_channel<VER>(c, b, k, pc[q], tkc[q], t4, Tb, iou_b, d0, d1, d2, d3, an, 0.f, r_b, part);
-            if (G) G[idx] = g * lp.inv_n;
+            if constexpr (HEAD) {
+              const float dt = head_act_grad(g * lp.inv_n, pc[q], k == 2 || k == 3);
+              amax = fmaxf(amax, fabsf(dt));
+              G[idx] = dt;
+            } else {
+              if (G) G[idx] = g * lp.inv_n;
+            }
           }
         }
       }
@@ -447,6 +493,35 @@
     const double s = red[threadIdx.x][0] + red[threadIdx.x][1] + red[threadIdx.x][2] + red[threadIdx.x][3];
     atomicAdd(&out[threadIdx.x], s * invN);
   }
+  if constexpr (HEAD) {
+    if (bound != nullptr) {
+      __shared__ float wmax[4];
+#pragma unroll
+      for (int o = 32; o > 0; o >>= 1) amax = fmaxf(amax, __shfl_xor(amax, o, 64));
+      if (lane == 0) wmax[wave] = amax;
+      __syncthreads();
+      if (threadIdx.x == 0) {
+        const float m = fmaxf(fmaxf(wmax[0], wmax[1]), fmaxf(wmax[2], wmax[3]));
+        if (__builtin_bit_cast(unsigned, m) > *reinterpret_cast<volatile unsigned*>(bound))
+          atomicMax(bound, __builtin_bit_cast(unsigned, m));
+      }
+    }
+  }
+}
+
+template <int VER, bool PREF>
+__global__ __launch_bounds__(256) void loss_kernel(const LossParams lp, const float* __restrict__ y_true,
+                                                   const float* __restrict__ y_pred, float* __restrict__ dpred,
+                                                   double* __restrict__ out) {
+  loss_body<VER, PREF, false>(lp, y_true, y_pred, dpred, out, nullptr, nullptr);
+}
+
+template <int VER>
+__global__ __launch_bounds__(256, 3) void loss_head_kernel(const LossParams lp, const float* __restrict__ y_true,
+                                                        const float* __restrict__ t, float* __restrict__ dt,
+                                                        double* __restrict__ out, const float* __restrict__ head_anchors,
+                                                        unsigned* __restrict__ bound) {
+  loss_body<VER, true, true>(lp, y_true, t, dt, out, head_anchors, bound);
 }
 
 template <int VER>
@@ -587,6 +662,42 @@
   return check_launch("loss_kernel");
 }
 
+extern "C" int yolo_loss_head_fwd_bwd(const yolo_loss_cfg* cfg, const float* y_true, const float* t,
+                                      const float* head_anchors, double* loss_out, float* dt, float grad_scale,
+                                      void* dy_planes, void* workspace, size_t workspace_bytes, void* stream) {
+  if (int rc = validate_cfg(cfg)) return rc;
+  YOLO_REQUIRE(y_true && t && head_anchors && loss_out && dt, "loss_head: null pointer");
+  YOLO_REQUIRE(cfg->version == 3 || cfg->version == 4, "loss_head: version %d has no logits form", cfg->version);
+  const int PD = cfg->A * (5 + cfg->C);
+  YOLO_REQUIRE(PD <= 256, "loss_head: %d prediction channels per cell, at most 256", PD);
+  LossParams lp;
+  lp.c = *cfg;
+  lp.cells = (long long)cfg->N * cfg->gh * cfg->gw;
+  lp.inv_n = grad_scale / (float)cfg->N;
+  lp.dec = (workspace != nullptr && workspace_bytes >= (size_t)lp.cells * 8) ? reinterpret_cast<int*>(workspace) : nullptr;
+  hipStream_t st = as_stream(stream);
+  if (hipMemsetAsync(loss_out, 0, 8 * sizeof(double), st) != hipSuccess) {
+    set_error("loss_head: memset failed");
+    return YOLO_ERR_LAUNCH;
+  }
+  unsigned* bound = nullptr;
+  if (dy_planes != nullptr) {
+    bound = reinterpret_cast<unsigned*>(reinterpret_cast<unsigned char*>(dy_planes) + planes_body_bytes(lp.cells, (PD + 15) / 16 * 16));
+    if (hipMemsetAsync(bound, 0, 16, st) != hipSuccess) {
+      set_error("loss_head: memset failed");
+      return YOLO_ERR_LAUNCH;
+    }
+  }
+  long long blocks = (lp.cells + 3) / 4;
+  if (blocks > 2048) blocks = 2048;
+  dim3 grid((unsigned)blocks), block(256);
+  if (cfg->version == 3)
+    hipLaunchKernelGGL(loss_head_kernel<3>, grid, block, 0, st, lp, y_true, t, dt, loss_out, head_anchors, bound);
+  else
+    hipLaunchKernelGGL(loss_head_kernel<4>, grid, block, 0, st, lp, y_true, t, dt, loss_out, head_anchors, bound);
+  return check_launch("loss_head_kernel");
+}
+
 extern "C" int yolo_metrics(const yolo_loss_cfg* cfg, const float* y_true, const float* y_pred, float recall_thresh,
                             double* out, void* stream) {
   if (int rc = validate_cfg(cfg)) return rc;
diff --git a/tf2_yolo_amd/engine.py b/tf2_yolo_amd/engine.py
--- a/tf2_yolo_amd/engine.py
+++ b/tf2_yolo_amd/engine.py
@@ -285,6 +285,7 @@
         self.batch = None
         self.act = {}
         self.training = False
+        self._head_logits = False
         self.grad_ready_hook = None
         self.backward_begin_hook = None
         self._infer_scale_valid = False
@@ -542,7 +543,9 @@
         self._wTp_valid = False
         self._infer_scale_valid = False
 
-    def forward(self, x, training=False, stop_after=None):
+    def forward(self, x, training=False, stop_after=None, head_logits=False):
+        if head_logits and not training:
+            raise YoloHipError("head_logits belongs to a training-mode forward")
         if x.dtype != torch.float32 or not x.is_cuda:
             raise YoloHipError("forward expects a float32 CUDA tensor")
         x = x.contiguous()
@@ -551,6 +554,7 @@
                                f"{(self.input.h, self.input.w, self.input.c)}")
         self.allocate(x.shape[0])
         self.training = training
+        self._head_logits = bool(head_logits)
         self.act[self.input.tid] = x
         self._xp_valid = set()
         self._tbound_set = set()
@@ -576,7 +580,13 @@
             fwd(u, training)
         if not training:
             self._infer_scale_valid = True
+        if head_logits:
+            return [t.producer.t for t in self.outputs]
         return [self.act[t.tid] for t in self.outputs]
+
+    def head_dy_planes(self, t):
+        u = t.producer
+        return self._dyp_own[u.name] if u.cpad else None
 
     def _prepare_filters(self, training):
         if training and self._overlap_wgrad and self._prep_beside and not (self._wp_valid and self._wT_valid and self._wTp_valid):
@@ -656,7 +666,8 @@
             ops.conv2d_fwd_head_unit(u.desc, self._xp(u.src), u.wp, bias, u.A, u.C, u.version, anchors, u.t, u.yact)
             return
         self._conv_fwd(u, bias, u.t)
-        ops.head_act_fwd(u.t, u.A, u.C, u.version, anchors, out=u.yact)
+        if not self._head_logits:
+            ops.head_act_fwd(u.t, u.A, u.C, u.version, anchors, out=u.yact)
 
     def _fwd_upsample(self, u, training):
         if not training and self._infer_small_fuse and self._concat_planes and u.out.tid in self._up_producer:
@@ -841,12 +852,18 @@
         self._filter_and_data_grad(u, dy, dyp, dbias, grads)
 
     def _bwd_head(self, u, dout, grads):
-        dt = ops.head_act_bwd(u.yact, dout, u.A, u.C, u.version, self._anchors_dev.get(u.name),
-                              danchors=self._anchor_grad_views.get(u.name) if self.anchors_trainable else None)
+        if self._head_logits:
+            dt = dout
+        else:
+            dt = ops.head_act_bwd(u.yact, dout, u.A, u.C, u.version, self._anchors_dev.get(u.name),
+                                  danchors=self._anchor_grad_views.get(u.name) if self.anchors_trainable else None)
         if not u.cpad:
             return self._filter_and_data_grad(u, dt, self._dyp(u, dt), self._gview(u.p_bias), grads)
         rows = self.batch * u.out.h * u.out.w
-        dtp = ops.split_planes_padded(dt, rows, u.out.c, out=self._next_dyp_buffer(u))
+        if self._head_logits:
+            dtp = ops.split_planes_padded_bounded(dt, rows, u.out.c, out=self._next_dyp_buffer(u))
+        else:
+            dtp = ops.split_planes_padded(dt, rows, u.out.c, out=self._next_dyp_buffer(u))
         with self._beside_backward(dt):
             ops.zero_bytes(u.dw_pad)
             ops.conv2d_wgrad_planes(u.desc_pad, self._xplanes[u.src.tid], dtp, u.dw_pad)
diff --git a/tf2_yolo_amd/model.py b/tf2_yolo_amd/model.py
--- a/tf2_yolo_amd/model.py
+++ b/tf2_yolo_amd/model.py
@@ -334,6 +334,28 @@
                 _ops.zero_bytes(self.net.grads)
             return None
 
+    def head_loss_plan(self, with_metrics=False):
+        from . import plan
+        net = self.net
+        metrics = with_metrics or any(self.metrics or [])
+        return plan.plan_head_loss(net.outputs, self.loss or [], net._opts, net.anchors_trainable, metrics)
+
+    def _forward_and_losses(self, x, y_list, with_metrics=False):
+        from . import ops
+        net = self.net
+        fused, _ = self.head_loss_plan(with_metrics)
+        outs = net.forward(x, training=True, head_logits=fused)
+        if self._dpred is None or self._dpred[0].shape != outs[0].shape:
+            self._dpred = [torch.empty_like(o) for o in outs]
+        for i, (t, o, yt) in enumerate(zip(net.outputs, outs, y_list)):
+            if fused:
+                lf = self.loss[i]
+                ops.loss_head_fwd_bwd(lf.cfg(o.shape[0]), yt, o, net._anchors_dev[t.producer.name], loss_out=self._loss_bufs[i],
+                                      dt=self._dpred[i], grad_scale=1.0, dy_planes=net.head_dy_planes(t))
+            else:
+                self.loss[i].fwd_bwd(yt, o, grad_scale=1.0, dpred=self._dpred[i], loss_out=self._loss_bufs[i])
+        return outs
+
     def train_step_device(self, x, y_list, with_metrics=False):
         if self.optimizer is None:
             raise YoloHipError("compile() the model before training")
@@ -342,11 +364,7 @@
             bufs = self._captured_step(x, y_list)
             if bufs is not None:
                 return bufs, None
-        outs = self.net.forward(x, training=True)
-        if self._dpred is None or self._dpred[0].shape != outs[0].shape:
-            self._dpred = [torch.empty_like(o) for o in outs]
-        for i, (o, yt) in enumerate(zip(outs, y_list)):
-            self.loss[i].fwd_bwd(yt, o, grad_scale=1.0, dpred=self._dpred[i], loss_out=self._loss_bufs[i])
+        outs = self._forward_and_losses(x, y_list, with_metrics)
         mvals = None
         if with_metrics:
             mvals = [[m(yt, o) for m in ms] for ms, o, yt in zip(self.metrics, outs, y_list)]
diff --git a/tf2_yolo_amd/ops.py b/tf2_yolo_amd/ops.py
--- a/tf2_yolo_amd/ops.py
+++ b/tf2_yolo_amd/ops.py
@@ -338,6 +338,18 @@
         raise YoloHipError("split_planes_padded: output buffer too small")
     check(_lib.load().yolo_split_planes_padded(_p(x), int(rows), int(c_src), int(c), _p(out), _stream()),
           "yolo_split_planes_padded")
+    return out
+
+
+def split_planes_padded_bounded(x, rows, c_src, out):
+    _chk_f32(x)
+    c = (c_src + 15) // 16 * 16
+    if x.numel() != rows * c_src:
+        raise YoloHipError("split_planes_padded_bounded: tensor size does not match rows x C_src")
+    if out.numel() < planes_bytes(rows, c) or out.dtype != torch.uint8:
+        raise YoloHipError("split_planes_padded_bounded: output buffer too small")
+    check(_lib.load().yolo_split_planes_padded_bounded(_p(x), int(rows), int(c_src), int(c), _p(out), _stream()),
+          "yolo_split_planes_padded_bounded")
     return out
 
 
@@ -984,6 +996,32 @@
     return loss_out, dpred
 
 
+def loss_head_fwd_bwd(cfg, y_true, t, anchors_dev, loss_out=None, dt=None, grad_scale=1.0, dy_planes=None, decisions=None):
+    _chk_f32(y_true, t, dt, anchors_dev)
+    cells, pd = cfg.N * cfg.gh * cfg.gw, cfg.A * (5 + cfg.C)
+    if cfg.version not in (3, 4) or pd > 256:
+        raise YoloHipError(f"loss_head: version {cfg.version} with {pd} channels per cell has no logits form")
+    if y_true.numel() != cells * (5 + cfg.C) or t.numel() != cells * pd:
+        raise YoloHipError(f"loss_head: tensor sizes do not match cfg (cells={cells}, C={cfg.C}, A={cfg.A})")
+    if anchors_dev is None or anchors_dev.numel() < 2 * cfg.A or not anchors_dev.is_contiguous():
+        raise YoloHipError(f"loss_head: need the head's {2 * cfg.A} anchor values as one contiguous CUDA tensor")
+    if loss_out is None:
+        loss_out = torch.empty(8, device=t.device, dtype=torch.float64)
+    if dt is None:
+        dt = torch.empty_like(t)
+    elif dt.numel() != t.numel():
+        raise YoloHipError("loss_head: dt does not have the size of t")
+    if dy_planes is not None and (dy_planes.dtype != torch.uint8 or dy_planes.numel() < planes_bytes(cells, (pd + 15) // 16 * 16)):
+        raise YoloHipError("loss_head: dy_planes is too small for the planes of dt")
+    if decisions is not None and (decisions.dtype != torch.int32 or decisions.numel() < 2 * cells or not decisions.is_cuda):
+        raise YoloHipError("loss_head: decisions must be an int32 CUDA tensor with 2 entries per cell")
+    check(_lib.load().yolo_loss_head_fwd_bwd(byref(cfg), _p(y_true), _p(t), _p(anchors_dev), _p(loss_out), _p(dt),
+                                             float(grad_scale), _p(dy_planes), _p(decisions),
+                                             0 if decisions is None else decisions.numel() * 4, _stream()),
+          "yolo_loss_head_fwd_bwd")
+    return loss_out, dt
+
+
 def metrics(cfg, y_true, y_pred, recall_thresh=0.5, out=None):
     _chk_f32(y_true, y_pred)
     if out is None:
diff --git a/tf2_yolo_amd/plan.py b/tf2_yolo_amd/plan.py
--- a/tf2_yolo_amd/plan.py
+++ b/tf2_yolo_amd/plan.py
@@ -32,6 +32,7 @@
         o.infer_onepass = on("YOLO_INFER_ONEPASS")
         o.infer_small_fuse = on("YOLO_INFER_SMALL_FUSE")
         o.dgrad_classes = on("YOLO_DGRAD_CLASSES")
+        o.head_loss_fuse = on("YOLO_HEAD_LOSS_FUSE")
         return o
 
 
@@ -196,6 +197,31 @@
     g.pred_total = 2 * max(len(units), 1)
 
 
+def plan_head_loss(outputs, losses, opts, anchors_trainable=False, with_metrics=False):
+    from .losses import YoloLoss
+    if not opts.head_loss_fuse:
+        return False, "switched off (YOLO_HEAD_LOSS_FUSE=0)"
+    if with_metrics:
+        return False, "metrics read the activated outputs"
+    if anchors_trainable:
+        return False, "trainable anchors need dL/dy"
+    if not outputs or len(losses) != len(outputs):
+        return False, "one loss per output is needed"
+    for t, lf in zip(outputs, losses):
+        u = t.producer
+        if u is None or u.kind != "head" or u.version not in (3, 4) or u.anchors is None:
+            return False, f"{t.name}: not a v3 / v4 head with anchors"
+        if u.cout > 256:
+            return False, f"{u.name}: {u.cout} channels per cell, at most 256"
+        if type(lf) is not YoloLoss or lf.version != u.version:
+            return False, f"{u.name}: the loss is not the library's own for version {u.version}"
+        if (lf.bbox_num, lf.class_num, lf.grid_shape) != (u.A, u.C, (u.out.h, u.out.w)):
+            return False, f"{u.name}: the loss was made for another grid, anchor count or class count"
+        if u.cpad and not opts.dyp_per_layer:
+            return False, f"{u.name}: padded head gradient planes in a shared buffer (YOLO_DYP_PER_LAYER=0)"
+    return True, ""
+
+
 def plan_batch(units, N, opts):
     b = SimpleNamespace(desc={}, desc_pad={}, pool_pad={}, xplanes_bytes={}, dyp_own_bytes={}, dyp_shared_bytes=0,
                         bnred_cap={})
```

After: 1102, median of 6. No clear change (+0.6%).
